# enijkamp/apex_example

Measured on AMD Instinct MI355X. Metric: images/sec (whole node) ResNet-50 amp O2, higher is better.
Workload: dtype bf16; 1 GPU; model=resnet50, global_batch=256, per_gpu_batch=256, image_size=224, parallelism=dp1, impl=amd, opt_level=O2, optimizer=FusedSGD(momentum=0.9, wd=5e-5), channels_last=True, fused_bn=True, syncbn=False, force_collectives=False, gemm_1x1=True, hip_graph=False, main_stream_priority=default, deterministic=False

## Files before the change

apex_example_amd/models/resnet.py:

```python
from __future__ import annotations

import weakref

import torch
import torch.nn as nn

from ..ops.batch_norm import BatchNorm2dReLU
from ..ops.batch_norm import bn_add_bn_relu
from ..ops.conv import Conv2d1x1, Conv2d3x3, StemConv2d, conv1x1_pair_s2
from ..ops.pool import (GlobalAvgPool2dNHWC, MaxPool2dNHWC, bn_relu_maxpool,
                        bn_relu_maxpool_fusable)


def conv3x3(in_planes, out_planes, stride=1, groups=1, dilation=1, mfma=False):
    if mfma and stride in (1, 2) and groups == 1 and dilation == 1:
        return Conv2d3x3(in_planes, out_planes, stride)
    return nn.Conv2d(in_planes, out_planes, kernel_size=3, stride=stride, padding=dilation,
                     groups=groups, bias=False, dilation=dilation)


def conv1x1(in_planes, out_planes, stride=1, gemm=False):
    if gemm:
        return Conv2d1x1(in_planes, out_planes, stride=stride)
    return nn.Conv2d(in_planes, out_planes, kernel_size=1, stride=stride, bias=False)
# ... 8 lines not shown
        if fused:
            self.bn = BatchNorm2dReLU(planes, fuse_relu=relu)
        else:
            self.bn = nn.BatchNorm2d(planes)
        if zero_init:
            nn.init.zeros_(self.bn.weight)

    def forward(self, x, z=None):
        if self.fused:
            return self.bn(x, z)
        y = self.bn(x)
        if z is not None:
            y = y + z
        return torch.relu(y) if self.relu_after else y


def _link_stats(conv, bnact):
    if bnact.fused:
        conv._amd_stats_bn = weakref.ref(bnact)


class BasicBlock(nn.Module):
    expansion = 1

    def __init__(self, inplanes, planes, stride=1, downsample=None, fused_bn=False,
                 zero_init_residual=False, gemm_1x1=False):
        super().__init__()
        self.conv1 = conv3x3(inplanes, planes, stride, mfma=gemm_1x1)
        self.bn1 = _BNAct(planes, True, fused_bn)
        self.conv2 = conv3x3(planes, planes, mfma=gemm_1x1)
        self.bn2 = _BNAct(planes, True, fused_bn, zero_init_residual)
        self.downsample = downsample
        _link_stats(self.conv1, self.bn1)
        _link_stats(self.conv2, self.bn2)

    def forward(self, x):
        identity = x if self.downsample is None else self.downsample(x)
        out = self.bn1(self.conv1(x))
        return self.bn2(self.conv2(out), identity)


class Bottleneck(nn.Module):
    expansion = 4

    def __init__(self, inplanes, planes, stride=1, downsample=None, fused_bn=False,
                 zero_init_residual=False, gemm_1x1=False):
        super().__init__()
        width = planes
        self.conv1 = conv1x1(inplanes, width, gemm=gemm_1x1)
        self.bn1 = _BNAct(width, True, fused_bn)
        self.conv2 = conv3x3(width, width, stride, mfma=gemm_1x1)
        self.bn2 = _BNAct(width, True, fused_bn)
        self.conv3 = conv1x1(width, planes * self.expansion, gemm=gemm_1x1)
        self.bn3 = _BNAct(planes * self.expansion, True, fused_bn, zero_init_residual)
        self.downsample = downsample
        _link_stats(self.conv1, self.bn1)
        _link_stats(self.conv2, self.bn2)
        _link_stats(self.conv3, self.bn3)

    def forward(self, x):
        fuse_ds = self.downsample is not None and self.bn3.fused and self.downsample.bn.fused
        proj = identity = None
        if (isinstance(self.conv1, Conv2d1x1) and self.downsample is not None
                and self.downsample.conv.stride == (2, 2)):
            out, proj = conv1x1_pair_s2(self.conv1, self.downsample.conv, x)
        elif isinstance(self.conv1, Conv2d1x1):
            out, skip = self.conv1.forward_with_skip(x)
            if self.downsample is None:
                identity = skip
            else:
                proj = self.downsample.conv(skip)
        else:
            if self.downsample is None:
                identity = x
            else:
                proj = self.downsample.conv(x)
            out = self.conv1(x)
        if proj is not None and not fuse_ds:
            identity = self.downsample.bn(proj)
        out = self.bn1(out)
        out = self.bn2(self.conv2(out))
        if proj is not None and fuse_ds:
            return bn_add_bn_relu(self.bn3.bn, self.conv3(out), self.downsample.bn.bn, proj)
        return self.bn3(self.conv3(out), identity)


class _Downsample(nn.Module):
    def __init__(self, inplanes, outplanes, stride, fused_bn, gemm_1x1=False):
        super().__init__()
        self.conv = conv1x1(inplanes, outplanes, stride, gemm=gemm_1x1)
        self.bn = _BNAct(outplanes, False, fused_bn)
        _link_stats(self.conv, self.bn)

    def forward(self, x):
        return self.bn(self.conv(x))


class ResNet(nn.Module):
    def __init__(self, block, layers, num_classes=1000, fused_bn=False, zero_init_residual=False,
                 gemm_1x1=False):
        super().__init__()
        self.fused_bn = fused_bn
        self.gemm_1x1 = gemm_1x1
        self.inplanes = 64
        if gemm_1x1 and self.inplanes == 64:
            self.conv1 = StemConv2d(3, self.inplanes)
        else:
            self.conv1 = nn.Conv2d(3, self.inplanes, kernel_size=7, stride=2, padding=3,
                                   bias=False)
        self.bn1 = _BNAct(self.inplanes, True, fused_bn)
        if isinstance(self.conv1, StemConv2d):
            _link_stats(self.conv1, self.bn1)
        pool = MaxPool2dNHWC if fused_bn else nn.MaxPool2d
        self.maxpool = pool(kernel_size=3, stride=2, padding=1)
        self.layer1 = self._make_layer(block, 64, layers[0], 1, zero_init_residual)
        self.layer2 = self._make_layer(block, 128, layers[1], 2, zero_init_residual)
        self.layer3 = self._make_layer(block, 256, layers[2], 2, zero_init_residual)
        self.layer4 = self._make_layer(block, 512, layers[3], 2, zero_init_residual)
        self.avgpool = GlobalAvgPool2dNHWC() if fused_bn else nn.AdaptiveAvgPool2d((1, 1))
        self.fc = nn.Linear(512 * block.expansion, num_classes)
        for m in self.modules():
            if isinstance(m, nn.Conv2d):
                nn.init.kaiming_normal_(m.weight, mode="fan_out", nonlinearity="relu")

    def _make_layer(self, block, planes, blocks, stride, zero_init_residual):
        downsample = None
        if stride != 1 or self.inplanes != planes * block.expansion:
            downsample = _Downsample(self.inplanes, planes * block.expansion, stride,
                                     self.fused_bn, self.gemm_1x1)
        layers = [block(self.inplanes, planes, stride, downsample, self.fused_bn,
                        zero_init_residual, self.gemm_1x1)]
        self.inplanes = planes * block.expansion
        for _ in range(1, blocks):
            layers.append(block(self.inplanes, planes, fused_bn=self.fused_bn,
                                zero_init_residual=zero_init_residual, gemm_1x1=self.gemm_1x1))
        return nn.Sequential(*layers)

    def forward(self, x):
        x = self.conv1(x)
        if (self.fused_bn and isinstance(self.maxpool, MaxPool2dNHWC)
                and bn_relu_maxpool_fusable(x, self.bn1.bn, self.maxpool)):
            x = bn_relu_maxpool(x, self.bn1.bn, self.maxpool)
        else:
            x = self.maxpool(self.bn1(x))
        x = self.layer1(x)
        x = self.layer2(x)
        x = self.layer3(x)
        x = self.layer4(x)
        x = self.avgpool(x)
        x = torch.flatten(x, 1)
        return self.fc(x)


def resnet18(**kw):
    return ResNet(BasicBlock, [2, 2, 2, 2], **kw)


def resnet34(**kw):
    return ResNet(BasicBlock, [3, 4, 6, 3], **kw)


def resnet50(**kw):
    return ResNet(Bottleneck, [3, 4, 6, 3], **kw)


def resnet101(**kw):
# ... 6 lines not shown
```

apex_example_amd/ops/batch_norm.py:

```python
from __future__ import annotations

import os
import threading

import torch
import torch.distributed as dist

from .. import _native
from . import _ddp_direct

_BWD_EPI = os.environ.get("APEX_AMD_CONV_BN_BWD", "1") == "1"
_TLS = threading.local()
FUSED_BWD_CALLS = [0]

_X2_BWD = os.environ.get("APEX_AMD_BN_X2", "1") == "1"
X2_BWD_CALLS = [0]


def _x2_target_ok(zc, ctx, weight):
    return (getattr(zc, "world", 0) == 1 and not getattr(zc, "fuse_relu", True)
            and not getattr(zc, "has_z", True) and getattr(zc, "count", -1) == ctx.count
            and not getattr(zc, "shape_channel_last", True) and not ctx.shape_channel_last
            and (zc.saved_tensors[2] is None) == (weight is None)
            and (weight is None or zc.saved_tensors[2].dtype == weight.dtype)
            and zc.saved_tensors[6] is None)


class BnBwdSrc:
    __slots__ = ("x", "mean", "invstd", "weight", "bias", "mask", "relu_mode", "result")

    def __init__(self, x, mean, invstd, weight, bias, mask, relu_mode):
        self.x, self.mean, self.invstd = x, mean, invstd
        self.weight, self.bias, self.mask, self.relu_mode = weight, bias, mask, relu_mode
        self.result = None


def _bwd_src(x, xl, mean, invstd, weight, bias, mask, fuse_relu, has_z):
    if not (_BWD_EPI and x.is_cuda and x.dtype == torch.bfloat16 and x.dim() == 4
            and x is xl and x.size(1) % 64 == 0
            and x.is_contiguous(memory_format=torch.channels_last)):
        return None
    if fuse_relu and has_z:
        if mask is None:
            return None
        mode = 1
    elif fuse_relu:
        if any(t is not None and t.dtype != torch.float32 for t in (weight, bias)):
            return None
        mode = 2
    else:
        mode = 0
    return BnBwdSrc(x, mean, invstd, weight, bias, mask, mode)


_RAW_RCCL = os.environ.get("APEX_AMD_SYNCBN_RAW_RCCL", "1") == "1"
_COMMS = {}


def _raw_comm(pg):
    return _raw_comm_rank(pg)[0]


def _raw_comm_rank(pg):
    if not _RAW_RCCL:
        return 0, -1
    c = _COMMS.get(id(pg))
    if c is not None and c[0] is pg:
        return c[1], c[2]
    from ..parallel.sync_batchnorm import is_syncbn_comm_group

    ptr = 0
    if is_syncbn_comm_group(pg) and _native.require().reducer.syncbn_raw_available():
        try:
            ptr = int(pg._get_backend(torch.device("cuda"))._comm_ptr())
        except Exception:
            ptr = 0
    rank = dist.get_rank(pg)
    if ptr:
        _COMMS[id(pg)] = (pg, ptr, rank)
    return ptr, rank


_SBN_EVENTS = None


def syncbn_timing(on=True):
    global _SBN_EVENTS
    _SBN_EVENTS = [] if on else None


def syncbn_timing_result():
    ev = _SBN_EVENTS
    if not ev:
        return None
    ev[-1][2].synchronize()
    out = {"calls": len(ev), "ms": 0.0, "allgather_ms": 0.0, "allreduce_ms": 0.0}
    for kind, a, b in ev:
        ms = a.elapsed_time(b)
        out["ms"] += ms
        out[kind + "_ms"] += ms
    return out


class _SbnTimer:
    def __init__(self, kind):
        self.kind = kind

    def __enter__(self):
        if _SBN_EVENTS is not None:
            self.a = torch.cuda.Event(enable_timing=True)
            self.a.record()
        return self

    def __exit__(self, *exc):
        if _SBN_EVENTS is not None and hasattr(self, "a"):
            b = torch.cuda.Event(enable_timing=True)
            b.record()
            _SBN_EVENTS.append((self.kind, self.a, b))
        return False


def _allreduce(t, pg):
    if t.is_cuda and _SBN_EVENTS is not None:
        with _SbnTimer("allreduce"):
            return _allreduce_body(t, pg)
    return _allreduce_body(t, pg)


def _allreduce_body(t, pg):
    if dist.get_backend(pg) == "nccl":
        comm = _raw_comm(pg)
        if comm:
            _native.require().reducer.syncbn_allreduce_raw(t, comm)
        else:
            _native.require().reducer.syncbn_allreduce(t, pg)
    else:
        dist.all_reduce(t, group=pg)


SLOT_GATHER_CALLS = [0]


def _gather_slot(C, world, rank, device):
    n = 2 * C + 1
    assert 0 <= rank < world, (rank, world)
    gathered = torch.empty(world * n, dtype=torch.float32, device=device)
    SLOT_GATHER_CALLS[0] += 1
    return gathered, gathered[rank * n:(rank + 1) * n]


def _direct_targets(params, need_w):
    direct = _ddp_direct.slots(*params) if need_w else None
    if direct is None:
        return None, None, None, True
    tw, aw = _ddp_direct.grad_target(params[0])
    tb, ab = _ddp_direct.grad_target(params[1])
    if aw != ab:
        return None, None, None, True
    return direct, tw, tb, aw


def bn_src_of(x):
    return getattr(x, "_amd_bn_src", None)


def _C():
    return _native.require().bn


def _to_logical(x, shape_channel_last):
    if shape_channel_last:
        C = x.size(-1)
        return x.reshape(-1, C)
    return x


class BatchNormFunction(torch.autograd.Function):
    @staticmethod
    def forward(ctx, x, z, weight, bias, running_mean, running_var, eps, momentum, process_group,
                fuse_relu, shape_channel_last, num_batches_tracked=None, force_collectives=False,
                slab=None, slab_shift=None):
        C = _C()
        ctx.params = (weight, bias)
        if ctx.needs_input_grad[2] or ctx.needs_input_grad[3]:
            _ddp_direct.note_use(weight, bias)
        orig_shape = x.shape
        xl = _to_logical(x, shape_channel_last)
        zl = _to_logical(z, shape_channel_last) if z is not None else None
        count = xl.numel() // xl.size(1)
        if process_group is False or not (dist.is_available() and dist.is_initialized()):
            world = 1
            force_collectives = False
        else:
            world = dist.get_world_size(process_group)
        collective = world > 1 or bool(force_collectives)
        want_mask = bool(fuse_relu) and zl is not None and xl.is_cuda
        if not collective and xl.is_cuda:
            if slab is not None:
                mean_g, invstd = C.slab_train_stats(slab, count, slab_shift, running_mean,
                                                    running_var, num_batches_tracked,
                                                    float(eps), float(momentum))
                if want_mask:
                    y, mask = C.apply_mask(xl, mean_g, invstd, weight, bias, zl, bool(fuse_relu))
                else:
                    y, mask = C.apply(xl, mean_g, invstd, weight, bias, zl, bool(fuse_relu)), None
            else:
                y, mean_g, invstd, mask = C.forward_local(xl, weight, bias, running_mean,
                                                          running_var, num_batches_tracked,
                                                          float(eps), float(momentum), zl,
                                                          bool(fuse_relu), want_mask)
            ctx.save_for_backward(xl, zl if mask is None else None, weight, bias, mean_g, invstd,
                                  mask)
            ctx.src = _TLS.src = _bwd_src(x, xl, mean_g, invstd, weight, bias, mask,
                                          bool(fuse_relu), zl is not None)
            ctx.pg, ctx.world, ctx.fuse_relu, ctx.total, ctx.count = None, 1, bool(fuse_relu), \
                None, count
            zg = getattr(z, "grad_fn", None) if z is not None else None
            ctx.zctx = zg if isinstance(zg, BatchNormFunction._backward_cls) else None
            ctx.pre = None
            ctx.orig_shape, ctx.has_z, ctx.shape_channel_last = orig_shape, z is not None, \
                shape_channel_last
            return y.view(orig_shape) if shape_channel_last else y
        if collective and xl.is_cuda:
            pg = process_group if process_group is not None else dist.group.WORLD
            nccl = dist.get_backend(pg) == "nccl"
            comm, rank = _raw_comm_rank(pg) if nccl else (0, dist.get_rank(pg))
            gathered = slot = None
            if comm or not nccl:
                gathered, slot = _gather_slot(xl.size(1), world, rank, x.device)
            packed = (C.slab_packed_stats(slab, count, slab_shift, out=slot) if slab is not None
                      else C.local_stats_packed(xl, out=slot))
            if nccl:
                R = _native.require().reducer
                with _SbnTimer("allgather"):
                    if comm:
                        mean_g, invstd, inv_total = R.syncbn_allgather_combine_raw(
                            packed, comm, world, float(eps), float(momentum), running_mean,
                            running_var, num_batches_tracked, gathered=gathered, rank=rank)
                    else:
                        mean_g, invstd, inv_total = R.syncbn_allgather_combine(
                            packed, pg, float(eps), float(momentum), running_mean,
                            running_var, num_batches_tracked)
            else:
                with _SbnTimer("allgather"):
                    dist.all_gather(list(gathered.chunk(world)), packed.clone(), group=pg)
                mean_g, invstd, inv_total = C.combine_stats_sync(
                    gathered.view(world, -1), float(eps), float(momentum), running_mean,
                    running_var, num_batches_tracked)
            if want_mask:
                y, mask = C.apply_mask(xl, mean_g, invstd, weight, bias, zl, bool(fuse_relu))
            else:
                y, mask = C.apply(xl, mean_g, invstd, weight, bias, zl, bool(fuse_relu)), None
            ctx.save_for_backward(xl, zl if mask is None else None, weight, bias, mean_g, invstd,
                                  mask)
            ctx.src = _TLS.src = _bwd_src(x, xl, mean_g, invstd, weight, bias, mask,
                                          bool(fuse_relu), zl is not None)
            ctx.pg, ctx.world, ctx.fuse_relu, ctx.total, ctx.count = pg, max(world, 2), \
                bool(fuse_relu), inv_total, count
            ctx.orig_shape, ctx.has_z, ctx.shape_channel_last = orig_shape, z is not None, \
                shape_channel_last
            return y.view(orig_shape) if shape_channel_last else y
        if num_batches_tracked is not None:
            num_batches_tracked.add_(1)
        mean, var = C.local_stats(xl)
        if collective:
            pg = process_group if process_group is not None else dist.group.WORLD
            cnt = torch.full((1,), float(count), dtype=torch.float32, device=x.device)
            packed = torch.cat([mean, var, cnt])
            gathered = torch.empty(world * packed.numel(), dtype=packed.dtype, device=x.device)
            dist.all_gather_into_tensor(gathered, packed, group=pg)
            g = gathered.view(world, -1)
            Cn = mean.numel()
            means, vars_, counts = g[:, :Cn], g[:, Cn:2 * Cn], g[:, 2 * Cn]
            total = counts.sum()
        else:
            pg = None
            means, vars_ = mean.view(1, -1), var.view(1, -1)
            counts = torch.full((1,), float(count), dtype=torch.float32, device=x.device)
            total = None
        mean_g, invstd, _ = C.combine_stats(means, vars_, counts, float(eps), float(momentum),
                                            running_mean, running_var)
        if want_mask:
            y, mask = C.apply_mask(xl, mean_g, invstd, weight, bias, zl, bool(fuse_relu))
        else:
            y, mask = C.apply(xl, mean_g, invstd, weight, bias, zl, bool(fuse_relu)), None
        ctx.save_for_backward(xl, zl if mask is None else None, weight, bias, mean_g, invstd, mask)
        ctx.src = None
        ctx.pg = pg
        ctx.world = max(world, 2) if collective else world
        ctx.fuse_relu = bool(fuse_relu)
        ctx.total = total
        ctx.count = count
        ctx.orig_shape = orig_shape
        ctx.has_z = z is not None
        ctx.shape_channel_last = shape_channel_last
        return y.view(orig_shape) if shape_channel_last else y

    @staticmethod
    def backward(ctx, dy):
        C = _C()
        xl, zl, weight, bias, mean, invstd, mask = ctx.saved_tensors
        dyl = _to_logical(dy, ctx.shape_channel_last)
        need_w = weight is not None and (ctx.needs_input_grad[2] or ctx.needs_input_grad[3])
        src = ctx.src
        res = src.result if src is not None else None
        if res is not None:
            src.result = None
        if res is not None and res[0] == dyl.data_ptr() and res[2] == dyl._version and (
                dyl.is_contiguous(memory_format=torch.channels_last)):
            FUSED_BWD_CALLS[0] += 1
            if ctx.world > 1:
                direct, tw, tb, acc = _direct_targets(ctx.params, need_w)
                sum_dy, sum_dy_xmu, gw, gb = C.slab_reduce_grad(res[1], invstd, weight, need_w,
                                                               sum_scale=ctx.total,
                                                               grad_weight=tw, grad_bias=tb,
                                                               accumulate=acc)
                if direct:
                    _ddp_direct.mark_ready(direct)
                    need_w = False
                n = sum_dy.numel()
                _allreduce(sum_dy.as_strided((2 * n,), (1,)), ctx.pg)
                total = 1.0
            else:
                sum_dy, sum_dy_xmu, gw, gb = C.slab_reduce_grad(res[1], invstd, weight, need_w)
                total = float(ctx.count)
            zc = getattr(ctx, "zctx", None) if ctx.has_z else None
            if _X2_BWD and zc is not None and ctx.world == 1 and _x2_target_ok(zc, ctx, weight):
                xd, _, wd, _, md, isd, _ = zc.saved_tensors
                if C.backward_x2_ok(dyl, xl, xd):
                    need_wd = wd is not None and (zc.needs_input_grad[2] or zc.needs_input_grad[3])
                    dx, s1, s2, gw2, gb2 = C.backward_elemt_x2(
                        dyl, xl, mean, invstd, weight, bias, sum_dy, sum_dy_xmu, total, xd, md,
                        isd, wd, need_wd)
                    zc.pre = (dyl.data_ptr(), dyl._version, s1, s2, gw2, gb2)
                    return (dx, dyl, gw if need_w else None, gb if need_w else None, None, None,
                            None, None, None, None, None, None, None, None, None)
            dx, _ = C.backward_elemt(dyl, xl, mean, invstd, weight, bias, sum_dy, sum_dy_xmu,
                                     total, None, False, False)
            return (dx, dyl if ctx.has_z else None, gw if need_w else None,
                    gb if need_w else None, None, None, None, None, None, None, None, None, None,
                    None, None)
        pre = getattr(ctx, "pre", None)
        if pre is not None:
            ctx.pre = None
            if pre[0] == dyl.data_ptr() and pre[1] == dyl._version:
                _, _, sum_dy, sum_dy_xmu, gw, gb = pre
                X2_BWD_CALLS[0] += 1
                dx, _ = C.backward_elemt(dyl, xl, mean, invstd, weight, bias, sum_dy, sum_dy_xmu,
                                         float(ctx.count), None, False, False)
                if ctx.shape_channel_last:
                    dx = dx.view(ctx.orig_shape)
                return (dx, None, gw if need_w else None, gb if need_w else None, None, None,
                        None, None, None, None, None, None, None, None, None)
        if ctx.world > 1 and xl.is_cuda:
            direct, tw, tb, acc = _direct_targets(ctx.params, need_w)
            sum_dy, sum_dy_xmu, gw, gb = C.reduce_grad(dyl, xl, mean, invstd, weight, bias, zl,
                                                       ctx.fuse_relu, need_w, mask=mask,
                                                       sum_scale=ctx.total, grad_weight=tw,
                                                       grad_bias=tb, accumulate=acc)
            if direct:
                _ddp_direct.mark_ready(direct)
                need_w = False
            n = sum_dy.numel()
            packed = sum_dy.as_strided((2 * n,), (1,))
            _allreduce(packed, ctx.pg)
            dx, dz = C.backward_elemt(dyl, xl, mean, invstd, weight, bias, sum_dy, sum_dy_xmu,
                                      1.0, zl, ctx.fuse_relu, ctx.has_z, mask=mask)
            if ctx.shape_channel_last:
                dx = dx.view(ctx.orig_shape)
                if dz is not None:
                    dz = dz.view(ctx.orig_shape)
            return (dx, dz if ctx.has_z else None, gw if need_w else None,
                    gb if need_w else None, None, None, None, None, None, None, None, None, None, None, None)
        if ctx.world == 1 and xl.is_cuda:
            dx, dz, gw, gb = C.backward_local(dyl, xl, mean, invstd, weight, bias, zl,
                                              ctx.fuse_relu, need_w, ctx.has_z, mask=mask)
            if ctx.shape_channel_last:
                dx = dx.view(ctx.orig_shape)
                if dz is not None:
                    dz = dz.view(ctx.orig_shape)
            return (dx, dz if ctx.has_z else None, gw if need_w else None,
                    gb if need_w else None, None, None, None, None, None, None, None, None, None, None, None)
        sum_dy, sum_dy_xmu, gw, gb = C.reduce_grad(dyl, xl, mean, invstd, weight, bias, zl,
                                                   ctx.fuse_relu, need_w, mask=mask)
        if ctx.world > 1:
            packed = torch.cat([sum_dy, sum_dy_xmu])
            dist.all_reduce(packed, group=ctx.pg)
            n = sum_dy.numel()
            packed = packed / ctx.total
            sum_dy, sum_dy_xmu = packed[:n], packed[n:]
            total = 1.0
        else:
            total = float(ctx.count)
        dx, dz = C.backward_elemt(dyl, xl, mean, invstd, weight, bias, sum_dy, sum_dy_xmu, total,
                                  zl, ctx.fuse_relu, ctx.has_z, mask=mask)
        if ctx.shape_channel_last:
            dx = dx.view(ctx.orig_shape)
            if dz is not None:
                dz = dz.view(ctx.orig_shape)
        return (dx, dz if ctx.has_z else None, gw if need_w else None, gb if need_w else None,
                None, None, None, None, None, None, None, None, None, None, None)


def take_slab(x, bn):
    ent = getattr(x, "_amd_bn_stats", None)
    if ent is None:
        return None, None
    del x._amd_bn_stats
    slab, shift, owner = ent
    if owner is not bn or slab.size(1) != x.size(1):
        return None, None
    return slab, shift


def batch_norm_act(x, weight, bias, running_mean, running_var, training, momentum, eps,
                   z=None, fuse_relu=False, process_group=False, shape_channel_last=False,
                   num_batches_tracked=None, force_collectives=False, slab=None, slab_shift=None):
    if training:
        _TLS.src = None
        y = BatchNormFunction.apply(x, z, weight, bias, running_mean, running_var, eps, momentum,
                                    process_group, fuse_relu, shape_channel_last,
                                    num_batches_tracked, force_collectives, slab, slab_shift)
        src = _TLS.src
        if src is not None:
            _TLS.src = None
            y._amd_bn_src = src
        return y
    if shape_channel_last:
        xs = x.movedim(-1, 1)
        zs = z.movedim(-1, 1) if z is not None else None
    else:
        xs, zs = x, z
    y = torch.nn.functional.batch_norm(xs, running_mean, running_var, weight, bias, False, 0.0, eps)
    if zs is not None:
        y = y + zs
    if fuse_relu:
        y = torch.relu(y)
    return y.movedim(1, -1) if shape_channel_last else y


class BatchNorm2dReLU(torch.nn.BatchNorm2d):

    def __init__(self, num_features, eps=1e-5, momentum=0.1, affine=True,
                 track_running_stats=True, fuse_relu=True, **kw):
        super().__init__(num_features, eps, momentum, affine, track_running_stats, **kw)
        self.fuse_relu = fuse_relu

    def _amd_accepts_slab(self):
        return self.training and (self.momentum is not None or not self.track_running_stats)

    def forward(self, x, z=None):
        slab, shift = take_slab(x, self)
        if not x.is_cuda and not _native.available():
            y = super().forward(x)
            if z is not None:
                y = y + z
            return torch.relu(y) if self.fuse_relu else y
        momentum = 0.0 if self.momentum is None else self.momentum
        nbt = None
        if self.training and self.track_running_stats:
            if self.momentum is None:
                self.num_batches_tracked.add_(1)
                momentum = 1.0 / float(self.num_batches_tracked)
            else:
                nbt = self.num_batches_tracked
        use_batch = self.training or not self.track_running_stats
        return batch_norm_act(x, self.weight, self.bias,
                              self.running_mean if self.track_running_stats else None,
                              self.running_var if self.track_running_stats else None,
                              use_batch, momentum, self.eps, z=z, fuse_relu=self.fuse_relu,
                              process_group=False, num_batches_tracked=nbt,
                              slab=slab if use_batch else None, slab_shift=shift)


_FUSE_DS = os.environ.get("APEX_AMD_BN_DS_FUSE", "1") == "1"
FUSED_DS_CALLS = [0]


class BatchNormAddBNReLUFunction(torch.autograd.Function):
    @staticmethod
    def forward(ctx, x, xd, w, b, wd, bd, rm, rv, nbt, rmd, rvd, nbtd, eps, mom, epsd, momd,
                slab, shift, slabd, shiftd):
        C = _C()
        ctx.params = (w, b, wd, bd)
        if ctx.needs_input_grad[2] or ctx.needs_input_grad[3]:
            _ddp_direct.note_use(w, b)
        if ctx.needs_input_grad[4] or ctx.needs_input_grad[5]:
            _ddp_direct.note_use(wd, bd)
        count = x.numel() // x.size(1)

        def stats(t, sl, sh, rm_, rv_, nbt_, eps_, mom_):
            if sl is not None:
                return C.slab_train_stats(sl, count, sh, rm_, rv_, nbt_, float(eps_), float(mom_))
            return C.train_stats(t, rm_, rv_, nbt_, float(eps_), float(mom_))

        mean, invstd = stats(x, slab, shift, rm, rv, nbt, eps, mom)
        meand, invstdd = stats(xd, slabd, shiftd, rmd, rvd, nbtd, epsd, momd)
        y, mask = C.apply2_mask(x, mean, invstd, w, b, xd, meand, invstdd, wd, bd)
        ctx.save_for_backward(x, xd, w, b, wd, bd, mean, invstd, meand, invstdd, mask)
        ctx.src = _TLS.src = _bwd_src(x, x, mean, invstd, w, b, mask, True, True)
        ctx.count = count
        FUSED_DS_CALLS[0] += 1
        return y

    @staticmethod
    def backward(ctx, dy):
        C = _C()
        x, xd, w, b, wd, bd, mean, invstd, meand, invstdd, mask = ctx.saved_tensors
        need = w is not None and (ctx.needs_input_grad[2] or ctx.needs_input_grad[3])
        needd = wd is not None and (ctx.needs_input_grad[4] or ctx.needs_input_grad[5])
        cnt = float(ctx.count)
        src = ctx.src
        res = src.result if src is not None else None
        if res is not None:
            src.result = None
        if (res is not None and res[0] == dy.data_ptr() and res[2] == dy._version
                and dy.is_contiguous(memory_format=torch.channels_last)):
            FUSED_BWD_CALLS[0] += 1
            s1, s2, gw, gb = C.slab_reduce_grad(res[1], invstd, w, need)
            dx, t1, t2, gwd, gbd = C.backward_elemt_x2(dy, x, mean, invstd, w, b, s1, s2, cnt,
                                                       xd, meand, invstdd, wd, needd)
            dxd, _ = C.backward_elemt(dy, xd, meand, invstdd, wd, bd, t1, t2, cnt, None, False,
                                      False)
        else:
            dyc = dy.contiguous(memory_format=torch.channels_last)
            s1, s2, gw, gb = C.reduce_grad(dyc, x, mean, invstd, w, b, None, True, need,
                                           mask=mask)
            dx, d = C.backward_elemt(dyc, x, mean, invstd, w, b, s1, s2, cnt, None, True, True,
                                     mask=mask)
            dxd, _, gwd, gbd = C.backward_local(d, xd, meand, invstdd, wd, bd, None, False,
                                                needd, False)
        return (dx, dxd, gw if need else None, gb if need else None, gwd if needd else None,
                gbd if needd else None) + (None,) * 14


def _ds_fusable(bn, x, bnd, xd):
    return (_FUSE_DS and type(bn) is BatchNorm2dReLU and type(bnd) is BatchNorm2dReLU
            and bn.training and bnd.training and bn.fuse_relu and not bnd.fuse_relu
            and bn.track_running_stats and bnd.track_running_stats
            and bn.momentum is not None and bnd.momentum is not None
            and bn.affine == bnd.affine and x.is_cuda and xd.is_cuda and x.dim() == 4
            and x.shape == xd.shape and x.dtype == xd.dtype
            and x.dtype in (torch.bfloat16, torch.float16)
            and (not bn.affine or bn.weight.dtype == bnd.weight.dtype)
            and _native.available() and _C().backward_x2_ok(x, x, xd))


def bn_add_bn_relu(bn, x, bnd, xd):
    if not _ds_fusable(bn, x, bnd, xd):
        return bn(x, bnd(xd))
    slab, shift = take_slab(x, bn)
    slabd, shiftd = take_slab(xd, bnd)
    _TLS.src = None
    y = BatchNormAddBNReLUFunction.apply(
        x, xd, bn.weight, bn.bias, bnd.weight, bnd.bias, bn.running_mean, bn.running_var,
# ... 8 lines not shown
```

apex_example_amd/ops/conv.py:

```python
from __future__ import annotations

import collections
import os
import threading

import torch
import torch.nn as nn
import torch.nn.functional as F

from .. import _native
from . import _ddp_direct
from .batch_norm import bn_src_of

_USE_WSTREAM = os.environ.get("APEX_AMD_WGRAD_STREAM", "1") == "1"
_SIDE = {}
_JOIN = {}
_LOCK = threading.Lock()


def _ddp_slot(p):
    return _ddp_direct.slot(p)


def _side_mode(params):
    ps = [p for p in params if p is not None]
    if not _USE_WSTREAM or not ps or not ps[0].is_cuda:
        return None
    if torch.cuda.is_current_stream_capturing():
        return None
    if all(p.grad is None for p in ps) and not any(
            getattr(p, "_amd_grad_is_bucket_view", False) for p in ps):
        import torch.distributed as dist
        if dist.is_available() and dist.is_initialized() and dist.get_world_size() > 1:
            return None
        return "free"
    if _DDP_SIDE and all(_ddp_slot(p) is not None for p in ps):
        return "ddp"
    return None


_DDP_SIDE = os.environ.get("APEX_AMD_WGRAD_STREAM_DDP", "1") == "1"
_SIDE_EVENTS = {}


_TEST_SIDE_SLEEP = 0


def _join_side():
    with _LOCK:
        pending = list(_JOIN.items())
        _JOIN.clear()
        for idx, _ in pending:
            _SIDE_EVENTS.pop(idx, None)
    for idx, (main, _task) in pending:
        for key, side in list(_SIDE.items()):
            if key[0] == idx:
                main.wait_stream(side)


def _lag_for(mode):
    return 4 if mode == "ddp" else 0


def join_side_streams():
    _join_side()


class _SideWgrad:

    def __init__(self, weight, *more, enable=True):
        self.params = (weight,) + more
        self.mode = _side_mode(self.params) if enable else None
        self.on = self.mode is not None
        if self.on:
            dev = weight.device
            self.main = torch.cuda.current_stream(dev)
            high = self.mode == "ddp"
            key = (dev.index, high)
            self.side = _SIDE.get(key)
            if self.side is None:
                prio = torch.cuda.Stream.priority_range()[1] if high else 0
                self.side = torch.cuda.Stream(dev, priority=prio)
                _SIDE[key] = self.side
            self.ev = self.main.record_event()

    def run(self, fn, *used):
        if not self.on:
            return fn()
        self.side.wait_event(self.ev)
        with torch.cuda.stream(self.side):
            if _TEST_SIDE_SLEEP:
                torch.cuda._sleep(_TEST_SIDE_SLEEP)
            dw = fn()
            outs = dw if isinstance(dw, tuple) else (dw,)
            if self.mode == "ddp":
# ... 142 lines not shown
            return got
        return _native.require().conv.transpose_weight(weight)
    return weight.reshape(co, ci).t().contiguous().view(ci, co, 1, 1)


def _conv1x1_dgrad(dy, weight, xshape):
    n, ci, h, w = xshape
    co = weight.shape[0]
    if _own_1x1(dy.dtype, co, ci, n * h * w) and weight.dtype == torch.bfloat16:
        return _native.require().conv.conv_fwd(dy, _transpose_1x1(weight), 1)
    dx2 = torch.mm(_as_rows(dy), weight.reshape(co, ci))
    return dx2.view(n, h, w, ci).permute(0, 3, 1, 2)


def _as_rows(t):
    n, c, h, w = t.shape
    return t.permute(0, 2, 3, 1).reshape(n * h * w, c)


_CONV_BN_STATS = os.environ.get("APEX_AMD_CONV_BN_STATS", "1") == "1"
_TLS = threading.local()


def _stats_bn(conv, x):
    if not (_CONV_BN_STATS and x.is_cuda and x.dtype == torch.bfloat16):
        return None
    link = getattr(conv, "_amd_stats_bn", None)
    owner = link() if link is not None else None
    bn = getattr(owner, "bn", None) if owner is not None else None
    if bn is None or not bn.training or not hasattr(bn, "_amd_accepts_slab"):
        return None
    if not bn._amd_accepts_slab():
        return None
    return bn


def _shift_of(bn):
    rm = bn.running_mean if bn.track_running_stats else None
    if rm is not None and rm.dtype == torch.float32 and rm.is_contiguous():
        return rm
    return None


def _conv_fwd(x, weight, stride, bn):
    cv = _native.require().conv
    if bn is None:
        return cv.conv_fwd(x, weight, stride)
    shift = _shift_of(bn)
    y, slab = cv.conv_fwd_stats(x, weight, stride, shift)
    _TLS.slab = (slab, shift, bn)
    return y


def _tag_stats(y):
    ent = getattr(_TLS, "slab", None)
    if ent is not None:
        _TLS.slab = None
        y._amd_bn_stats = ent
    return y




_BNBWD_MAX_M = int(os.environ.get("APEX_AMD_BNBWD_MAX_M", str((1 << 31) - 1)))
_BNBWD_S2 = os.environ.get("APEX_AMD_BNBWD_S2", "0") == "1"


def _bnbwd_ok(dy, weight, src, xshape, has_add=False):
    m = xshape[0] * xshape[2] * xshape[3]
    return (src is not None and dy.is_cuda and dy.dtype == torch.bfloat16
            and weight.dtype == torch.bfloat16 and tuple(src.x.shape) == tuple(xshape)
            and dy.size(1) % 64 == 0 and xshape[1] % 64 == 0 and m < (1 << 31)
            and (has_add or m <= _BNBWD_MAX_M) and _native.available())


def _dgrad_bn(dy, wprep, add, src, add_stride2=False):
    g, slab = _native.require().conv.conv_fwd_bnbwd(
        dy, wprep, add, src.x, src.mask, src.mean, src.invstd, src.weight, src.bias,
        src.relu_mode, add_stride2)
    src.result = (g.data_ptr(), slab, g._version)
    return g


class Conv1x1GemmFunction(torch.autograd.Function):
    @staticmethod
    def forward(ctx, x, weight, bn=None, src=None):
        ctx.save_for_backward(x, weight)
        ctx.src = src
        if ctx.needs_input_grad[1]:
            _ddp_direct.note_use(weight)
        n, ci, h, w = x.shape
        if ctx.needs_input_grad[0] and weight.dtype == torch.bfloat16 and (
                src is not None or _own_1x1(x.dtype, weight.shape[0], ci, n * h * w)):
            _register_prep(weight)
        return _conv1x1_fwd(x, weight, bn)

    @staticmethod
    def backward(ctx, dy):
        x, weight = ctx.saved_tensors
        dy = dy.contiguous(memory_format=torch.channels_last)
        dx = dw = None
        side = _SideWgrad(weight) if ctx.needs_input_grad[1] else None
        if ctx.needs_input_grad[0]:
            if _bnbwd_ok(dy, weight, ctx.src, x.shape):
                dx = _dgrad_bn(dy, _transpose_1x1(weight), None, ctx.src)
            else:
                dx = _conv1x1_dgrad(dy, weight, x.shape)
        ctx.src = None
        if ctx.needs_input_grad[1]:
            direct = None if side.on else _ddp_direct.slots(weight)
            tgt, acc = _ddp_direct.grad_target(weight) if direct is not None else (None, True)
            if direct is not None and tgt.is_contiguous():
                wgrad_1x1(_as_rows(dy), _as_rows(x), weight.dtype, out=tgt, accumulate=acc)
                _ddp_direct.mark_ready(direct)
            else:
                so, sa = _side_out(side, weight)
                dw = side.run(lambda: _wgrad_1x1_w(dy, x, weight, so, sa), dy, x)
        return dx, dw, None, None


class Conv1x1SkipFunction(torch.autograd.Function):

    @staticmethod
    def forward(ctx, x, weight, bn=None, src=None):
        ctx.save_for_backward(x, weight)
        ctx.src = src
        if ctx.needs_input_grad[1]:
            _ddp_direct.note_use(weight)
        if src is not None and ctx.needs_input_grad[0] and weight.dtype == torch.bfloat16:
            _register_prep(weight)
        return _conv1x1_fwd(x, weight, bn), x.view_as(x)

    @staticmethod
    def backward(ctx, dy, dskip):
        x, weight = ctx.saved_tensors
        n, ci, h, w = x.shape
        co = weight.shape[0]
        dx = dw = None
        if dy is not None:
            dy = dy.contiguous(memory_format=torch.channels_last)
        side = _SideWgrad(weight) if (ctx.needs_input_grad[1] and dy is not None) else None
        src, ctx.src = ctx.src, None
        if ctx.needs_input_grad[0]:
            if dy is None:
                dx = dskip
            elif _bnbwd_ok(dy, weight, src, x.shape, has_add=dskip is not None) and (
                    dskip is None or (dskip.dtype == torch.bfloat16 and dskip.shape == x.shape)):
                add = (dskip.contiguous(memory_format=torch.channels_last)
                       if dskip is not None else None)
                dx = _dgrad_bn(dy, _transpose_1x1(weight), add, src)
            else:
                w2 = weight.reshape(co, ci)
                if dskip is not None:
                    dskip = dskip.contiguous(memory_format=torch.channels_last)
                    dx2 = _as_rows(dskip).addmm_(_as_rows(dy), w2)
                else:
                    dx2 = torch.mm(_as_rows(dy), w2)
                dx = dx2.view(n, h, w, ci).permute(0, 3, 1, 2)
        if ctx.needs_input_grad[1] and dy is not None:
            direct = None if side.on else _ddp_direct.slots(weight)
            tgt, acc = _ddp_direct.grad_target(weight) if direct is not None else (None, True)
            if direct is not None and tgt.is_contiguous():
                wgrad_1x1(_as_rows(dy), _as_rows(x), weight.dtype, out=tgt, accumulate=acc)
                _ddp_direct.mark_ready(direct)
            else:
                so, sa = _side_out(side, weight)
                dw = side.run(lambda: _wgrad_1x1_w(dy, x, weight, so, sa), dy, x)
        return dx, dw, None, None


class Conv1x1Stride2Function(torch.autograd.Function):

    @staticmethod
    def forward(ctx, x, weight, bn=None):
        ctx.save_for_backward(x, weight)
        if ctx.needs_input_grad[1]:
            _ddp_direct.note_use(weight)
        if ctx.needs_input_grad[0]:
            _register_prep(weight)
        return _conv_fwd(x, weight, 2, bn)

    @staticmethod
    def backward(ctx, dy):
        x, weight = ctx.saved_tensors
        cv = _native.require().conv
        dy = dy.contiguous(memory_format=torch.channels_last)
        co, ci = weight.shape[0], weight.shape[1]
        dx = dw = None
        side = _SideWgrad(weight) if ctx.needs_input_grad[1] else None
        if ctx.needs_input_grad[0]:
            dx = cv.conv_dgrad_s2(dy, _transpose_1x1(weight), x.size(2), x.size(3))
        if ctx.needs_input_grad[1]:
            direct = None if side.on else _ddp_direct.slots(weight)
            tgt, acc = _ddp_direct.grad_target(weight) if direct is not None else (None, True)
            if direct is not None and tgt.is_contiguous(memory_format=torch.channels_last):
                cv.conv_wgrad(dy, x, weight.dtype, 0, 2, 1, out=tgt, accumulate=acc)
                _ddp_direct.mark_ready(direct)
            else:
                so, sa = _side_out(side, weight, cl=True)
                dw = side.run(lambda: cv.conv_wgrad(dy, x, weight.dtype, 0, 2, 1, out=so,
                                                    accumulate=sa), dy, x)
# ... 26 lines not shown
        return y1, yd

    @staticmethod
    def backward(ctx, dy1, dyd):
        x, w1, wd = ctx.saved_tensors
        n, ci, h, w = x.shape
        cv = _native.require().conv
        src, ctx.src = ctx.src, None
        dx = dw1 = dwd = None
        if dy1 is not None:
            dy1 = dy1.contiguous(memory_format=torch.channels_last)
        if dyd is not None:
            dyd = dyd.contiguous(memory_format=torch.channels_last)
        side1 = _SideWgrad(w1) if (ctx.needs_input_grad[1] and dy1 is not None) else None
        sided = _SideWgrad(wd) if (ctx.needs_input_grad[2] and dyd is not None) else None
        if ctx.needs_input_grad[0]:
            cd = (_conv1x1_dgrad(dyd, wd, (n, ci, h // 2, w // 2)).contiguous(
                memory_format=torch.channels_last) if dyd is not None else None)
            if dy1 is None:
                dx = torch.zeros_like(x)
                if cd is not None:
                    dx[:, :, ::2, ::2] = cd
            elif cd is not None and _bnbwd_ok(dy1, w1, src, x.shape, has_add=True):
                PAIR_S2_CALLS[0] += 1
                dx = _dgrad_bn(dy1, _transpose_1x1(w1), cd, src, add_stride2=True)
            else:
                dx = _conv1x1_dgrad(dy1, w1, x.shape).contiguous(
                    memory_format=torch.channels_last)
                if cd is not None:
                    dx[:, :, ::2, ::2] += cd
        if side1 is not None:
            direct = None if side1.on else _ddp_direct.slots(w1)
            tgt, acc = _ddp_direct.grad_target(w1) if direct is not None else (None, True)
            if direct is not None and tgt.is_contiguous():
                wgrad_1x1(_as_rows(dy1), _as_rows(x), w1.dtype, out=tgt, accumulate=acc)
                _ddp_direct.mark_ready(direct)
            else:
                so, sa = _side_out(side1, w1)
                dw1 = side1.run(lambda: _wgrad_1x1_w(dy1, x, w1, so, sa), dy1, x)
        if sided is not None:
            direct = None if sided.on else _ddp_direct.slots(wd)
            tgt, acc = _ddp_direct.grad_target(wd) if direct is not None else (None, True)
            if direct is not None and tgt.is_contiguous(memory_format=torch.channels_last):
                cv.conv_wgrad(dyd, x, wd.dtype, 0, 2, 1, out=tgt, accumulate=acc)
                _ddp_direct.mark_ready(direct)
            else:
                so, sa = _side_out(sided, wd, cl=True)
                dwd = sided.run(lambda: cv.conv_wgrad(dyd, x, wd.dtype, 0, 2, 1, out=so,
                                                      accumulate=sa), dyd, x)
        return dx, dw1, dwd, None, None, None


def conv1x1_pair_s2(conv1, convd, x):
    if (_PAIR_S2 and isinstance(conv1, Conv2d1x1) and isinstance(convd, Conv2d1x1)
            and conv1._gemm_ok(x) and convd._strided_ok(x) and x.dtype == torch.bfloat16
            and conv1.weight.dtype == torch.bfloat16 and _native.available()):
        y1, yd = Conv1x1PairS2Function.apply(x, conv1.weight, convd.weight,
                                             _stats_bn(conv1, x), _stats_bn(convd, x),
                                             bn_src_of(x))
        ent1, ent2 = getattr(_TLS, "pair", (None, None))
        _TLS.pair = (None, None)
        if ent1 is not None:
            y1._amd_bn_stats = ent1
        if ent2 is not None:
            yd._amd_bn_stats = ent2
        return y1, yd
    return conv1(x), convd(x)


class Conv2d1x1(nn.Conv2d):

    def __init__(self, in_planes, out_planes, stride=1, bias=False):
        super().__init__(in_planes, out_planes, kernel_size=1, stride=stride, bias=bias)

    def forward(self, x):
        if self._gemm_ok(x):
            return _tag_stats(Conv1x1GemmFunction.apply(x, self.weight, _stats_bn(self, x),
                                                        bn_src_of(x)))
        if self._strided_ok(x):
            return _tag_stats(Conv1x1Stride2Function.apply(x, self.weight, _stats_bn(self, x)))
        return F.conv2d(x, self.weight, self.bias, self.stride, self.padding, self.dilation,
                        self.groups)

    def forward_with_skip(self, x):
        if self._gemm_ok(x):
            y, skip = Conv1x1SkipFunction.apply(x, self.weight, _stats_bn(self, x),
                                                bn_src_of(x))
            return _tag_stats(y), skip
        return self.forward(x), x

    def _strided_ok(self, x):
        return (self.stride == (2, 2) and self.bias is None and x.is_cuda and x.dim() == 4
                and x.dtype == torch.bfloat16 and self.weight.dtype == torch.bfloat16
                and x.is_contiguous(memory_format=torch.channels_last) and self.groups == 1
                and x.size(2) % 2 == 0 and x.size(3) % 2 == 0
                and x.size(0) * x.size(2) * x.size(3) < (1 << 22)
                and self.in_channels % 64 == 0 and self.out_channels % 64 == 0)

    def _gemm_ok(self, x):
        return (self.stride == (1, 1) and self.bias is None and x.is_cuda and x.dim() == 4
                and x.is_contiguous(memory_format=torch.channels_last)
                and x.dtype == self.weight.dtype and self.groups == 1)


_WGRAD3 = "tap"
_WGRAD64 = True
_WGRAD9_ALL = os.environ.get("APEX_AMD_WGRAD9", "0") == "1"


def _wgrad3_algo(x, weight, stride):
    cin, cout = x.size(1), weight.size(0)
    if not (_WGRAD64 and stride == 1 and x.size(3) <= 56 and cin % 64 == 0
            and cout % 64 == 0):
        return 0
    if cin == 64 and cout == 64:
        return 4
    return 4 if _WGRAD9_ALL and x.size(3) >= 14 else 0
_USE_SPLITK_REDUCE = True
_USE_ROT_KERNEL = True


def _rot_weight(weight):
    if _USE_ROT_KERNEL and weight.is_cuda and weight.element_size() == 2:
        got = _prepared(weight)
        if got is not None:
            return got
        return _native.require().conv.rot_weight(weight)
    return weight.flip(2, 3).transpose(0, 1).contiguous(memory_format=torch.channels_last)


_USE_PREP = True
_PREP_PENDING = {}
_PREP_READY = {}


def _register_prep(weight):
    if not (_USE_PREP and weight.is_cuda and weight.element_size() == 2):
        return
    k = id(weight)
    _PREP_READY.pop(k, None)
    _PREP_PENDING[k] = weight


def _prepared(weight):
    k = id(weight)
    ent = _PREP_READY.get(k)
    if ent is not None and ent[0] is weight:
        return ent[1]
    if k not in _PREP_PENDING:
        return None
    ws = list(_PREP_PENDING.values())
    _PREP_PENDING.clear()
    _PREP_READY.clear()
    outs = _native.require().conv.prep_weights(ws)
    for w, o in zip(ws, outs):
        _PREP_READY[id(w)] = (w, o)
    return _PREP_READY[k][1]


class Conv3x3Function(torch.autograd.Function):

    @staticmethod
    def forward(ctx, x, weight, stride, bn=None, src=None):
        ctx.save_for_backward(x, weight)
        ctx.stride = stride
        ctx.src = src if stride == 1 else None
# ... 127 lines not shown
```

csrc/hip/bn_nhwc.hip:

```cpp
#include <cstdio>
#include <cstdlib>

#include "bn_common.h"

namespace amd {

namespace {

struct NGeom {
  int ctile, rows_iter, cblocks;
};

NGeom ngeom(int64_t C, bool vec) {
  NGeom g;
  int64_t cv = vec ? C / 8 : C;
  g.ctile = (int)(cv < 64 ? cv : 64);
  if (g.ctile < 1) g.ctile = 1;
  g.rows_iter = kBNThreads / g.ctile;
  g.cblocks = (int)((cv + g.ctile - 1) / g.ctile);
  return g;
}

}

// ... 132 lines not shown
  float k[W], s1[W], s2[W];
#pragma unroll
  for (int i = 0; i < W; ++i) k[i] = s1[i] = s2[i] = 0.f;
  if (active) {
    ldw<T, W>(x + c0, k);
    for (int64_t r = r0 + ri; r < r1; r += (int64_t)rows_iter * U) {
      float v[U][W];
#pragma unroll
      for (int u = 0; u < U; ++u) {
        const int64_t rr = r + (int64_t)u * rows_iter;
#pragma unroll
        for (int i = 0; i < W; ++i) v[u][i] = k[i];
        if (rr < r1) ldw<T, W>(x + rr * C + c0, v[u]);
      }
#pragma unroll
      for (int u = 0; u < U; ++u)
#pragma unroll
        for (int i = 0; i < W; ++i) {
          const float d = v[u][i] - k[i];
          s1[i] += d;
          s2[i] = fmaf(d, d, s2[i]);
        }
    }
  }
  block_slab_write<W>(s1, s2, ci, ri, ctile, rows_iter, c0, C, slab);
}

constexpr int kBNBlockChans = 64 * 8;

template <typename F>
__device__ __forceinline__ void stage_params(int C, int cb, int n, F&& f) {
  const int lim = cb + n < C ? n : C - cb;
  for (int k = threadIdx.x; k < lim; k += blockDim.x) f(cb + k, k);
  __syncthreads();
}

template <typename T, typename TW, bool VEC, int U, bool ZZ, bool ZA = false>
__global__ void __launch_bounds__(kBNThreads)
    apply_k(const T* __restrict__ x, const float* __restrict__ mean,
            const float* __restrict__ invstd, const TW* __restrict__ w, const TW* __restrict__ b,
            const T* __restrict__ z, T* __restrict__ y, uint8_t* __restrict__ rmask, int64_t M,
            int C, int ctile, int rows_iter, int relu, const float* __restrict__ meanz = nullptr,
            const float* __restrict__ invstdz = nullptr, const TW* __restrict__ wz = nullptr,
            const TW* __restrict__ bz = nullptr) {
  constexpr int W = VEC ? 8 : 1;
  const int Cb = C >> 3;
  const int ci = threadIdx.x % ctile, ri = threadIdx.x / ctile;
  const int c0 = (blockIdx.y * ctile + ci) * W;
  __shared__ __attribute__((aligned(16))) float s_par[ZA ? 4 : 2][kBNBlockChans];
  const int cb = blockIdx.y * ctile * W;
  stage_params(C, cb, ctile * W, [&](int c, int k) {
    chan_affine(mean, invstd, wload(w, c, 1.f), wload(b, c, 0.f), c, s_par[0][k], s_par[1][k]);
    if constexpr (ZA)
      chan_affine(meanz, invstdz, wload(wz, c, 1.f), wload(bz, c, 0.f), c, s_par[ZA ? 2 : 0][k],
                  s_par[ZA ? 3 : 1][k]);
  });
  if (ri >= rows_iter || c0 >= C) return;
  float sc[W], sh[W], scz[W], shz[W];
#pragma unroll
  for (int i = 0; i < W; ++i) {
    sc[i] = s_par[0][c0 - cb + i];
    sh[i] = s_par[1][c0 - cb + i];
    scz[i] = ZA ? s_par[ZA ? 2 : 0][c0 - cb + i] : 0.f;
    shz[i] = ZA ? s_par[ZA ? 3 : 1][c0 - cb + i] : 0.f;
  }
  const int64_t stride = (int64_t)gridDim.x * rows_iter;
  for (int64_t r = (int64_t)blockIdx.x * rows_iter + ri; r < M; r += stride * U) {
    float v[U][W], zz[U][W];
#pragma unroll
    for (int u = 0; u < U; ++u) {
      const int64_t rr = r + (int64_t)u * stride;
      const int64_t rc = rr < M ? rr : M - 1;
      ldw<T, W>(x + rc * C + c0, v[u]);
      if constexpr (ZZ) ldw<T, W>(z + rc * C + c0, zz[u]);
    }
    asm volatile("" ::: "memory");
#pragma unroll
    for (int u = 0; u < U; ++u) {
      const int64_t rr = r + (int64_t)u * stride;
      if (rr >= M) continue;
      uint32_t mb = 0;
#pragma unroll
      for (int i = 0; i < W; ++i) {
        float o = fmaf(v[u][i], sc[i], sh[i]);
        if constexpr (ZA) {
          o += to_f32(from_f32<T>(fmaf(zz[u][i], scz[i], shz[i])));
        } else if constexpr (ZZ) {
          o += zz[u][i];
        }
        mb |= (o > 0.f ? 1u : 0u) << i;
        v[u][i] = relu ? fmaxf(o, 0.f) : o;
      }
      stw<T, W>(y + rr * C + c0, v[u]);
      if constexpr (W == 8) {
        if (rmask) rmask[rr * Cb + (c0 >> 3)] = (uint8_t)mb;
      }
    }
  }
}

template <typename T, typename TW, bool VEC, int U, int RM>
__global__ void __launch_bounds__(kBNThreads)
    reduce_k(const T* __restrict__ dy, const T* __restrict__ x, const float* __restrict__ mean,
             const float* __restrict__ invstd, const TW* __restrict__ w, const TW* __restrict__ b,
             const T* __restrict__ z, const uint8_t* __restrict__ rmask, int64_t M,
             int C, int ctile, int rows_iter, float* __restrict__ slab) {
  constexpr int W = VEC ? 8 : 1;
  const int Cb = C >> 3;
  const int ci = threadIdx.x % ctile, ri = threadIdx.x / ctile;
  const int c0 = (blockIdx.y * ctile + ci) * W;
  const bool active = ri < rows_iter && c0 < C;
  const int64_t per = (M + gridDim.x - 1) / gridDim.x;
  const int64_t r0 = (int64_t)blockIdx.x * per;
  const int64_t r1 = r0 + per < M ? r0 + per : M;
  float mu[W], sc[W], sh[W], s1[W], s2[W];
#pragma unroll
  for (int i = 0; i < W; ++i) mu[i] = sc[i] = sh[i] = s1[i] = s2[i] = 0.f;
  __shared__ __attribute__((aligned(16))) float s_par[3][kBNBlockChans];
  const int cb = blockIdx.y * ctile * W;
  stage_params(C, cb, ctile * W, [&](int c, int k) {
    s_par[0][k] = mean[c];
    chan_affine(mean, invstd, wload(w, c, 1.f), wload(b, c, 0.f), c, s_par[1][k], s_par[2][k]);
  });
  if (active) {
#pragma unroll
    for (int i = 0; i < W; ++i) {
      const int k = c0 - cb + i;
      mu[i] = s_par[0][k];
      sc[i] = s_par[1][k];
      sh[i] = s_par[2][k];
    }
    for (int64_t r = r0 + ri; r < r1; r += (int64_t)rows_iter * U) {
      float xv[U][W], dv[U][W], zv[U][W];
      uint32_t mk[U];
      bool ok[U];
#pragma unroll
      for (int u = 0; u < U; ++u) {
        const int64_t rr = r + (int64_t)u * rows_iter;
        ok[u] = rr < r1;
        const int64_t rc = ok[u] ? rr : r1 - 1;
        ldw<T, W>(x + rc * C + c0, xv[u]);
        ldw<T, W>(dy + rc * C + c0, dv[u]);
        mk[u] = 0;
        if constexpr (RM == 1) mk[u] = rmask[rc * Cb + (c0 >> 3)];
        if constexpr (RM == 2) ldw<T, W>(z + rc * C + c0, zv[u]);
      }
#pragma unroll
      for (int u = 0; u < U; ++u)
#pragma unroll
        for (int i = 0; i < W; ++i) {
          float d = dv[u][i];
          if constexpr (RM == 1) {
            d = ((mk[u] >> ((c0 + i) & 7)) & 1u) ? d : 0.f;
          } else if constexpr (RM >= 2) {
            float o = fmaf(xv[u][i], sc[i], sh[i]);
            if constexpr (RM == 2) o += zv[u][i];
            d = o > 0.f ? d : 0.f;
          }
          d = ok[u] ? d : 0.f;
          const float xe = ok[u] ? xv[u][i] : 0.f;
          s1[i] += d;
          s2[i] = fmaf(d, xe - mu[i], s2[i]);
        }
    }
  }
  block_slab_write<W>(s1, s2, ci, ri, ctile, rows_iter, c0, C, slab);
}

template <typename T, typename TW, bool VEC, int U, int RM, bool X2 = false>
__global__ void __launch_bounds__(kBNThreads)
    backward_k(const T* __restrict__ dy, const T* __restrict__ x, const float* __restrict__ mean,
               const float* __restrict__ invstd, const TW* __restrict__ w,
               const TW* __restrict__ b, const float* __restrict__ sum_dy,
               const float* __restrict__ sum_dy_xmu, float inv_n,
               const T* __restrict__ z, const uint8_t* __restrict__ rmask, T* __restrict__ dx,
               T* __restrict__ dz, int64_t M, int C, int ctile, int rows_iter,
               const T* __restrict__ x2 = nullptr, const float* __restrict__ mean2 = nullptr,
               float* __restrict__ slab2 = nullptr) {
  constexpr int W = VEC ? 8 : 1;
  const int Cb = C >> 3;
  const int ci = threadIdx.x % ctile, ri = threadIdx.x / ctile;
  const int c0 = (blockIdx.y * ctile + ci) * W;
  __shared__ __attribute__((aligned(16))) float s_par[X2 ? 6 : 5][kBNBlockChans];
  const int cb = blockIdx.y * ctile * W;
  stage_params(C, cb, ctile * W, [&](int c, int k) {
    const float wc = wload(w, c, 1.f);
    chan_affine(mean, invstd, wc, wload(b, c, 0.f), c, s_par[0][k], s_par[1][k]);
    const float is = invstd[c];
    const float mdy = sum_dy[c] * inv_n, mdyx = sum_dy_xmu[c] * inv_n;
    const float q1 = is * wc, q2 = -is * is * is * wc * mdyx;
    s_par[2][k] = q1;
    s_par[3][k] = q2;
    s_par[4][k] = -is * wc * mdy - q2 * mean[c];
    if constexpr (X2) s_par[X2 ? 5 : 0][k] = mean2[c];
  });
  float t1[W], t2[W], m2[W];
#pragma unroll
  for (int i = 0; i < W; ++i) t1[i] = t2[i] = m2[i] = 0.f;
  const bool active = ri < rows_iter && c0 < C;
  if (!X2 && !active) return;
  float sc[W], sh[W], k1[W], k2[W], k3[W];
#pragma unroll
  for (int i = 0; i < W; ++i) {
    const int k = active ? c0 - cb + i : 0;
    sc[i] = s_par[0][k];
    sh[i] = s_par[1][k];
    k1[i] = s_par[2][k];
    k2[i] = s_par[3][k];
    k3[i] = s_par[4][k];
    if constexpr (X2) m2[i] = s_par[X2 ? 5 : 0][k];
  }
  const int64_t stride = (int64_t)gridDim.x * rows_iter;
  for (int64_t r = (int64_t)blockIdx.x * rows_iter + ri; active && r < M; r += stride * U) {
    float xv[U][W], dv[U][W], zv[U][W], x2v[X2 ? U : 1][W];
    uint32_t mk[U];
#pragma unroll
    for (int u = 0; u < U; ++u) {
      const int64_t rr = r + (int64_t)u * stride;
      const int64_t rc = rr < M ? rr : M - 1;
      mk[u] = 0;
      ldw<T, W>(x + rc * C + c0, xv[u]);
      ldw<T, W>(dy + rc * C + c0, dv[u]);
      if constexpr (RM == 1) mk[u] = rmask[rc * Cb + (c0 >> 3)];
      if constexpr (RM == 2) ldw<T, W>(z + rc * C + c0, zv[u]);
      if constexpr (X2) ldw<T, W>(x2 + rc * C + c0, x2v[u]);
    }
    asm volatile("" ::: "memory");
#pragma unroll
    for (int u = 0; u < U; ++u) {
      const int64_t rr = r + (int64_t)u * stride;
      if (rr >= M) continue;
#pragma unroll
      for (int i = 0; i < W; ++i) {
        float d = dv[u][i];
        if constexpr (RM == 1) {
          d = ((mk[u] >> ((c0 + i) & 7)) & 1u) ? d : 0.f;
        } else if constexpr (RM >= 2) {
          float o = fmaf(xv[u][i], sc[i], sh[i]);
          if constexpr (RM == 2) o += zv[u][i];
          d = o > 0.f ? d : 0.f;
        }
        dv[u][i] = d;
        xv[u][i] = fmaf(d, k1[i], fmaf(xv[u][i], k2[i], k3[i]));
        if constexpr (X2) {
          t1[i] += d;
          t2[i] = fmaf(d, x2v[u][i] - m2[i], t2[i]);
        }
      }
      stw<T, W>(dx + rr * C + c0, xv[u]);
      if (dz) stw<T, W>(dz + rr * C + c0, dv[u]);
    }
  }
  if constexpr (X2) block_slab_write_cm<W>(t1, t2, ci, ri, ctile, rows_iter, c0, C, slab2);
}


constexpr int kSlabPerThread = 16;

static int slab_ch(int S) {
  int ch = 1;
  while (ch < 32 && (int64_t)S * ch * 2 <= (int64_t)kBNThreads * kSlabPerThread) ch *= 2;
  return ch;
}

template <int CH>
__device__ __forceinline__ void slab_t_sum(const float* __restrict__ slab, int S, int C, int c0,
                                           float* out) {
  constexpr int TPC = kBNThreads / CH;
  __shared__ float red[2][kBNThreads];
  const int k = threadIdx.x / TPC, t = threadIdx.x - k * TPC;
  const int c = c0 + k;
  float a[8], b[8];
#pragma unroll
  for (int u = 0; u < 8; ++u) a[u] = b[u] = 0.f;
  if (c < C) {
    const float* r0 = slab + (int64_t)c * S;
    const float* r1 = slab + (int64_t)(C + c) * S;
    int s = t;
    for (; s + 7 * TPC < S; s += 8 * TPC) {
      float va[8], vb[8];
#pragma unroll
      for (int u = 0; u < 8; ++u) {
        va[u] = r0[s + u * TPC];
        vb[u] = r1[s + u * TPC];
      }
#pragma unroll
      for (int u = 0; u < 8; ++u) {
        a[u] += va[u];
        b[u] += vb[u];
      }
    }
    for (; s < S; s += TPC) {
      a[0] += r0[s];
      b[0] += r1[s];
    }
  }
  red[0][threadIdx.x] = ((a[0] + a[1]) + (a[2] + a[3])) + ((a[4] + a[5]) + (a[6] + a[7]));
  red[1][threadIdx.x] = ((b[0] + b[1]) + (b[2] + b[3])) + ((b[4] + b[5]) + (b[6] + b[7]));
  __syncthreads();
#pragma unroll
  for (int w = TPC / 2; w > 0; w >>= 1) {
    if (t < w) {
      red[0][threadIdx.x] += red[0][threadIdx.x + w];
      red[1][threadIdx.x] += red[1][threadIdx.x + w];
    }
    __syncthreads();
  }
  if (t == 0) {
    out[k] = red[0][threadIdx.x];
    out[CH + k] = red[1][threadIdx.x];
  }
  __syncthreads();
}

template <int CH>
__global__ void __launch_bounds__(kBNThreads)
    slab_stats_k(const float* __restrict__ slab, int S, int C, int64_t count,
                 const float* __restrict__ shift, BNStatsOut out) {
  __shared__ float sums[2 * CH];
  const int c0 = blockIdx.x * CH;
  slab_t_sum<CH>(slab, S, C, c0, sums);
  const int k = threadIdx.x;
  if (k < CH && c0 + k < C) {
    const int c = c0 + k;
    const float sh = shift ? shift[c] : 0.f;
    const double m = (double)sums[k] / (double)count;
// ... 298 lines not shown
```

csrc/hip/conv_igemm.hip:

```cpp
#include <algorithm>
#include <cstdlib>
#include <cstring>
#include <type_traits>

#include "amd_dev.h"
#include "amd_kernels.h"

namespace amd {

namespace {

typedef float f32x4_t __attribute__((ext_vector_type(4)));

constexpr int kCT = 256;
constexpr int kBM = 128;
constexpr int kBK = 64;
constexpr int kRowBytes = kBK * 2;

__device__ uint4 g_zero16[4];

__device__ __forceinline__ int swz(int row, int chunk) {
  return row * kRowBytes + ((chunk ^ ((row >> 1) & 7)) << 4);
}

template <int RB>
__device__ __forceinline__ int swz_key(int row) {
  if constexpr (RB == 128) return (row >> 1) & 7;
  else return ((row >> 2) & 1) << 1;
}
template <int RB>
__device__ __forceinline__ int swzr(int row, int chunk) {
  return row * RB + ((chunk ^ swz_key<RB>(row)) << 4);
}

__device__ __forceinline__ void glds16(const void* g, unsigned char* l) {
  __builtin_amdgcn_global_load_lds((const __attribute__((address_space(1))) void*)g,
                                   (__attribute__((address_space(3))) void*)l, 16, 0, 0);
}

__device__ __forceinline__ void glds16a(const void* g, unsigned char* l) {
#if defined(__HIP_DEVICE_COMPILE__)
  const uint32_t la = (uint32_t)(uintptr_t)(__attribute__((address_space(3))) unsigned char*)l;
  asm volatile("global_load_lds_dwordx4 %0, off" : : "v"(g), "{m0}"(la) : "memory");
#endif
}

__device__ __forceinline__ void lds_barrier() {
  asm volatile("s_waitcnt lgkmcnt(0)" ::: "memory");
  __builtin_amdgcn_s_barrier();
  asm volatile("" ::: "memory");
}

__device__ __forceinline__ int xcd_remap(int bid, int nwg) {
  const int xcd = bid % 8, q = nwg / 8, r = nwg % 8;
  const int base = xcd < r ? xcd * (q + 1) : r * (q + 1) + (xcd - r) * q;
  return base + bid / 8;
}

enum ConvMode { kFwd3 = 0, kFwd1 = 1, kDgrad3 = 2, kDgrad1 = 3 };

template <int MODE>
__device__ __forceinline__ int conv_ntaps(int z) {
  if constexpr (MODE == kFwd3) return 9;
  else if constexpr (MODE == kFwd1) return 1;
  else if constexpr (MODE == kDgrad3) return ((z >> 1) ? 2 : 1) * ((z & 1) ? 2 : 1);
  else return z == 0 ? 1 : 0;
}

template <int MODE>
__device__ __forceinline__ void conv_tap(int z, int t, int& dh, int& dw, int& wt) {
  if constexpr (MODE == kFwd3) {
    const int r = t / 3, s = t - r * 3;
    dh = r - 1; dw = s - 1; wt = t;
  } else if constexpr (MODE == kDgrad3) {
    const int ph = z >> 1, pw = z & 1, ns = pw ? 2 : 1;
    const int ri = t / ns, si = t - ri * ns;
    const int r = ph ? 2 * ri : 1, s = pw ? 2 * si : 1;
    dh = (ph + 1 - r) >> 1; dw = (pw + 1 - s) >> 1;
    wt = 8 - (3 * r + s);
  } else {
    dh = 0; dw = 0; wt = 0;
  }
}

struct ConvGeom {
  int GH, GW, AH, AW, as, YH, YW, ys, KC, NC, M, kb_stride;
};

template <int BM, int BN, int CT = kCT>
// ... 64 lines not shown
      const int h = rem / g.GW, w = rem - h * g.GW;
      aoff = ((int64_t)(n * (g.GH >> 1) + (h >> 1)) * (g.GW >> 1) + (w >> 1)) * NC + c0;
      a_on = ((h | w) & 1) == 0;
    }
    P.av[q] = *reinterpret_cast<const uint4*>(a_on ? addp + aoff : zb);
    P.xv[q] = *reinterpret_cast<const uint4*>(x_on ? xp + off : zb);
    P.mk[q] = *(rm1 ? ep.rmask + opix * (NC >> 3) + (c0 >> 3) : g_ff16);
  }
}

template <int MODE, int BM, int BN, int CT, int RM, bool ADD, int TS>
__device__ __forceinline__ void bnbwd_store_t(const bf16_t* T, bf16_t* __restrict__ y,
                                              const ConvGeom& g, int m0, int n0, int z,
                                              const BnPre<BM, BN, CT>& P, float (&s1)[8],
                                              float (&s2)[8]) {
  using PT = BnPre<BM, BN, CT>;
  const int tid = threadIdx.x;
  const int cc = tid % PT::CPR, rg = tid / PT::CPR;
  const int c0 = n0 + cc * 8;
  __builtin_amdgcn_s_waitcnt(0x0F70);
  float sc[8], sh[8];
#pragma unroll
  for (int i = 0; i < 8; ++i) {
    sc[i] = P.iv[i] * P.wv[i];
    sh[i] = P.bv[i] - P.mu[i] * sc[i];
  }
#pragma unroll
  for (int q = 0; q < PT::ROWS; ++q) {
    const int row = q * PT::RGS + rg;
    const int m = m0 + row;
    if (m >= g.M) continue;
    const uint4 tv = *reinterpret_cast<const uint4*>(T + row * TS + cc * 8);
    const unsigned tw[4] = {tv.x, tv.y, tv.z, tv.w};
    const unsigned aw[4] = {P.av[q].x, P.av[q].y, P.av[q].z, P.av[q].w};
    const unsigned xw[4] = {P.xv[q].x, P.xv[q].y, P.xv[q].z, P.xv[q].w};
    unsigned ow[4];
#pragma unroll
    for (int k = 0; k < 4; ++k) {
      float o[2], xx[2];
      o[0] = __uint_as_float(tw[k] << 16);
      o[1] = __uint_as_float(tw[k] & 0xffff0000u);
      if constexpr (ADD) {
        o[0] += __uint_as_float(aw[k] << 16);
        o[1] += __uint_as_float(aw[k] & 0xffff0000u);
      }
      xx[0] = __uint_as_float(xw[k] << 16);
      xx[1] = __uint_as_float(xw[k] & 0xffff0000u);
      unsigned short hb[2];
#pragma unroll
      for (int h = 0; h < 2; ++h) {
        const int i = 2 * k + h;
        bool keep = true;
        if constexpr (RM == 1) keep = (P.mk[q] >> i) & 1u;
        else if constexpr (RM == 2) keep = fmaf(xx[h], sc[i], sh[i]) > 0.f;
        const bf16_t gb = (bf16_t)(keep ? o[h] : 0.f);
        const float gv = (float)gb;
        s1[i] += gv;
        s2[i] = fmaf(gv, xx[h] - P.mu[i], s2[i]);
        hb[h] = __builtin_bit_cast(unsigned short, gb);
      }
      ow[k] = (unsigned)hb[0] | ((unsigned)hb[1] << 16);
    }
    *reinterpret_cast<uint4*>(y + out_pix<MODE>(g, m, z) * g.NC + c0) =
        make_uint4(ow[0], ow[1], ow[2], ow[3]);
  }
}

template <int MODE, int BM, int BN, int CT, int TS>
__device__ __forceinline__ void bnbwd_store(const bf16_t* T, bf16_t* __restrict__ y,
                                            const ConvGeom& g, const ConvBnEpi& ep, int m0,
                                            int n0, int z, const BnPre<BM, BN, CT>& P,
                                            float (&s1)[8], float (&s2)[8]) {
  const bool add = ep.add != nullptr;
  switch (ep.relu_mode * 2 + (add ? 1 : 0)) {
    case 0: bnbwd_store_t<MODE, BM, BN, CT, 0, false, TS>(T, y, g, m0, n0, z, P, s1, s2); break;
    case 1: bnbwd_store_t<MODE, BM, BN, CT, 0, true, TS>(T, y, g, m0, n0, z, P, s1, s2); break;
    case 2: bnbwd_store_t<MODE, BM, BN, CT, 1, false, TS>(T, y, g, m0, n0, z, P, s1, s2); break;
    case 3: bnbwd_store_t<MODE, BM, BN, CT, 1, true, TS>(T, y, g, m0, n0, z, P, s1, s2); break;
    case 4: bnbwd_store_t<MODE, BM, BN, CT, 2, false, TS>(T, y, g, m0, n0, z, P, s1, s2); break;
    default: bnbwd_store_t<MODE, BM, BN, CT, 2, true, TS>(T, y, g, m0, n0, z, P, s1, s2); break;
  }
}

template <int MODE, int BM, int BN, int WM, int WN, int NB, int EPI = 0, int CT = kCT,
          int BK = kBK, bool EARLY = false>
__global__ void __launch_bounds__(CT, (NB * (BM + BN) * BK * 2 > 80 * 1024)
                                          ? 1 : (NB == 1 && EPI == 0 ? 3 : 2))
    conv_tap_k(const bf16_t* __restrict__ x, const bf16_t* __restrict__ wt,
               bf16_t* __restrict__ y, ConvGeom g, float* __restrict__ slab,
               const float* __restrict__ shift, ConvBnEpi ep) {
  constexpr int NW = CT / 64;
  static_assert(WM * WN == NW, "one wave per output sub-tile");
  constexpr int TM = BM / WM, TN = BN / WN;
  constexpr int FM = TM / 16, FN = TN / 16;
  constexpr int RB = BK * 2;
  constexpr int LPR = RB / 16;
  constexpr int RPI = 64 / LPR;
  constexpr int KS = BK / 32;
  constexpr int A_BYTES = BM * RB, B_BYTES = BN * RB;
  constexpr int BUF = A_BYTES + B_BYTES;
  constexpr int AI = BM / (RPI * NW);
  constexpr int BI = BN / (RPI * NW);
  static_assert(AI >= 1 && BI >= 1, "tile rows per wave");
  constexpr int G = AI + BI;
  constexpr int TS = BN + 8;
  constexpr int EPI_BYTES = BM * TS * 2 > 2 * CT * 8 * 4 ? BM * TS * 2 : 2 * CT * 8 * 4;
  constexpr int LDS_BYTES = NB * BUF > EPI_BYTES ? NB * BUF : EPI_BYTES;
  __shared__ __attribute__((aligned(1024))) unsigned char lds[LDS_BYTES];

  const int tid = threadIdx.x, lane = tid & 63, wid = tid >> 6;
  const int wm = wid / WN, wn = wid % WN;
  const int NTf = gridDim.y == 1 ? g.NC / BN : 1;
  const int lt = xcd_remap(blockIdx.x, gridDim.x);
  const int mt = lt / NTf, MTn = (int)gridDim.x / NTf;
  const int m0 = mt * BM, n0 = (gridDim.y == 1 ? lt - mt * NTf : (int)blockIdx.y) * BN;
  const int z = MODE == kDgrad3 ? (int)gridDim.z - 1 - (int)blockIdx.z : (int)blockIdx.z;
  const int ntaps = conv_ntaps<MODE>(z);
  const int KC = g.KC, M = g.M, GHW = g.GH * g.GW;

  const int lrow = lane / LPR, pchunk = lane % LPR;
  const bf16_t* abase[AI];
  unsigned amask[AI];
#pragma unroll
  for (int q = 0; q < AI; ++q) {
    const int row = wid * (BM / NW) + q * RPI + lrow;
    const int ch = pchunk ^ swz_key<RB>(row);
    const int m = m0 + row;
    const int mm = m < M ? m : 0;
    const int n = mm / GHW;
    const int rem = mm - n * GHW;
    const int gh = rem / g.GW, gw = rem - gh * g.GW;
    const int h = gh * g.as, w = gw * g.as;
    abase[q] = x + ((int64_t)(n * g.AH + h) * g.AW + w) * KC + ch * 8;
    unsigned mk = 0;
    constexpr int TMAX = MODE == kFwd3 ? 9 : (MODE == kDgrad3 ? 4 : 1);
#pragma unroll
    for (int t = 0; t < TMAX; ++t) {
      int dh, dw, wti;
      conv_tap<MODE>(z, t, dh, dw, wti);
      const int hh = h + dh, ww = w + dw;
      if (t < ntaps && m < M && hh >= 0 && hh < g.AH && ww >= 0 && ww < g.AW) mk |= 1u << t;
    }
    amask[q] = mk;
  }
  const bf16_t* bbase[BI];
#pragma unroll
  for (int q = 0; q < BI; ++q) {
    const int row = wid * (BN / NW) + q * RPI + lrow;
    bbase[q] = wt + (int64_t)(n0 + row) * g.kb_stride + (pchunk ^ swz_key<RB>(row)) * 8;
  }
  const int kc_per_tap = KC / BK;
  const int KT = ntaps * kc_per_tap;

#define CONV_ISSUE(kt_)                                                                     \
  {                                                                                         \
                                 \
    const int tap_ = (MODE == kFwd1 || MODE == kDgrad1) ? 0 : (kt_) / kc_per_tap;           \
    const int c0_ = ((kt_) - tap_ * kc_per_tap) * BK;                                       \
    int dh_, dw_, wt_;                                                                      \
    conv_tap<MODE>(z, tap_, dh_, dw_, wt_);                                                 \
    const int64_t aoff_ = (int64_t)(dh_ * g.AW + dw_) * KC + c0_;                           \
    const int boff_ = wt_ * KC + c0_;                                                       \
    unsigned char* A_ = lds + ((kt_) % NB) * BUF;                                           \
    unsigned char* B_ = A_ + A_BYTES;                                                       \
    _Pragma("unroll") for (int q = 0; q < AI; ++q) {                                        \
      const bool ok = (amask[q] >> tap_) & 1u;                                              \
      glds16(ok ? (const void*)(abase[q] + aoff_) : (const void*)g_zero16,                  \
             A_ + (wid * (BM / NW) + q * RPI) * RB);                                       \
    }                                                                                       \
    _Pragma("unroll") for (int q = 0; q < BI; ++q)                                          \
      glds16(bbase[q] + boff_, B_ + (wid * (BN / NW) + q * RPI) * RB);                      \
  }

  f32x4_t acc[FM][FN];
#pragma unroll
  for (int i = 0; i < FM; ++i)
#pragma unroll
    for (int j = 0; j < FN; ++j) acc[i][j] = f32x4_t{0.f, 0.f, 0.f, 0.f};

  const int fr = lane & 15, fg = lane >> 4;
  constexpr int CPR = BN / 8;
  const bool want_stats = EPI == 1 ? slab != nullptr
                                   : (MODE == kFwd3 || MODE == kFwd1) && slab != nullptr;
  const int scc = tid % CPR;
  float shv[8];
#pragma unroll
  for (int i = 0; i < 8; ++i)
    shv[i] = (EPI == 0 && want_stats && shift) ? shift[n0 + scc * 8 + i] : 0.f;

  BnPre<BM, BN, CT> pre;
  if constexpr (EPI == 1 && EARLY) bnbwd_prefetch<MODE, BM, BN, CT>(g, ep, m0, n0, z, pre);

  {
  #pragma unroll
    for (int p = 0; p < NB - 1; ++p)
      if (p < KT) CONV_ISSUE(p);

    for (int kt = 0; kt < KT; ++kt) {
      if constexpr (NB == 1) {
        if (kt > 0) __syncthreads();
        CONV_ISSUE(kt);
        asm volatile("s_waitcnt vmcnt(0)" ::: "memory");
        __builtin_amdgcn_s_barrier();
      } else {
        if (kt + NB - 2 < KT) {
          asm volatile("s_waitcnt vmcnt(%0)" ::"n"(G * (NB > 2 ? NB - 2 : 0)) : "memory");
        } else {
          asm volatile("s_waitcnt vmcnt(0)" ::: "memory");
        }
        __builtin_amdgcn_s_barrier();
        asm volatile("" ::: "memory");
        if (kt + NB - 1 < KT) CONV_ISSUE(kt + NB - 1);
      }
      const unsigned char* A = lds + (kt % NB) * BUF;
      const unsigned char* B = A + A_BYTES;
  #pragma unroll
      for (int ks = 0; ks < KS; ++ks) {
        const int ch = ks * 4 + fg;
        bf16x8 af[FM], bfr[FN];
  #pragma unroll
        for (int i = 0; i < FM; ++i)
          af[i] = *reinterpret_cast<const bf16x8*>(A + swzr<RB>(wm * TM + i * 16 + fr, ch));
  #pragma unroll
        for (int j = 0; j < FN; ++j)
          bfr[j] = *reinterpret_cast<const bf16x8*>(B + swzr<RB>(wn * TN + j * 16 + fr, ch));
  #pragma unroll
        for (int i = 0; i < FM; ++i)
  #pragma unroll
          for (int j = 0; j < FN; ++j)
            acc[i][j] = __builtin_amdgcn_mfma_f32_16x16x32_bf16(bfr[j], af[i], acc[i][j], 0, 0, 0);
      }
    }
  }
#undef CONV_ISSUE
  if constexpr (EPI == 1) {
    if constexpr (!EARLY) bnbwd_prefetch<MODE, BM, BN, CT>(g, ep, m0, n0, z, pre);
    lds_barrier();
  } else {
    __syncthreads();
  }

  bf16_t* T = reinterpret_cast<bf16_t*>(lds);
#pragma unroll
  for (int i = 0; i < FM; ++i)
#pragma unroll
    for (int j = 0; j < FN; ++j) {
      const int row = wm * TM + i * 16 + fr;
      const int col = wn * TN + j * 16 + fg * 4;
      const unsigned lo = (unsigned)__builtin_bit_cast(unsigned short, (bf16_t)acc[i][j][0]) |
                          ((unsigned)__builtin_bit_cast(unsigned short, (bf16_t)acc[i][j][1]) << 16);
      const unsigned hi = (unsigned)__builtin_bit_cast(unsigned short, (bf16_t)acc[i][j][2]) |
                          ((unsigned)__builtin_bit_cast(unsigned short, (bf16_t)acc[i][j][3]) << 16);
      *reinterpret_cast<uint2*>(T + row * TS + col) = make_uint2(lo, hi);
    }
  if constexpr (EPI == 1) {
    lds_barrier();
  } else {
    __syncthreads();
  }
  constexpr bool dense = MODE == kFwd3 || MODE == kFwd1;
  float s1[8], s2[8];
#pragma unroll
  for (int i = 0; i < 8; ++i) s1[i] = s2[i] = 0.f;
  if constexpr (EPI == 1) {
    bnbwd_store<MODE, BM, BN, CT, TS>(T, y, g, ep, m0, n0, z, pre, s1, s2);
  } else
  for (int c = tid; c < BM * CPR; c += CT) {
    const int row = c / CPR, cc = c - row * CPR;
    const int m = m0 + row;
    if (m >= M) continue;
    int64_t opix = m;
    if (!dense) {
      const int n = m / GHW;
      const int rem = m - n * GHW;
      const int gh = rem / g.GW, gw = rem - gh * g.GW;
      opix = (int64_t)(n * g.YH + gh * g.ys + (z >> 1)) * g.YW + gw * g.ys + (z & 1);
    }
    const uint4 v = *reinterpret_cast<const uint4*>(T + row * TS + cc * 8);
    *reinterpret_cast<uint4*>(y + opix * g.NC + n0 + cc * 8) = v;
    if (want_stats) {
      const unsigned wv[4] = {v.x, v.y, v.z, v.w};
#pragma unroll
      for (int q = 0; q < 4; ++q) {
        const float lo = __uint_as_float(wv[q] << 16) - shv[2 * q];
        const float hi = __uint_as_float(wv[q] & 0xffff0000u) - shv[2 * q + 1];
        s1[2 * q] += lo;
        s2[2 * q] = fmaf(lo, lo, s2[2 * q]);
        s1[2 * q + 1] += hi;
        s2[2 * q + 1] = fmaf(hi, hi, s2[2 * q + 1]);
      }
    }
  }
  if (want_stats) {
    constexpr int RGS = CT / CPR;
    lds_barrier();
    float* red = reinterpret_cast<float*>(lds);
    const int rg = tid / CPR;
#pragma unroll
    for (int i = 0; i < 8; ++i) {
      red[rg * BN + scc * 8 + i] = s1[i];
      red[RGS * BN + rg * BN + scc * 8 + i] = s2[i];
    }
    lds_barrier();
    if (tid < BN) {
      float a = 0.f, b = 0.f;
#pragma unroll 4
      for (int q = 0; q < RGS; ++q) {
        a += red[q * BN + tid];
        b += red[RGS * BN + q * BN + tid];
      }
      const int64_t S = (int64_t)MTn * gridDim.z, s = (int64_t)z * MTn + mt;
      slab[(int64_t)(n0 + tid) * S + s] = a;
      slab[(int64_t)(g.NC + n0 + tid) * S + s] = b;
    }
  }
}

int g_bnbwd_early = 1;

int g_conv_nfast = 1;

inline dim3 conv_grid(int mtiles, int ntiles, int nclasses, bool one_by_one) {
  (void)one_by_one;
  const bool fold = ntiles > 1 && (g_conv_nfast == 2 ||
                                   (g_conv_nfast == 1 && !(ntiles == 4 && mtiles >= 1024)));
  return fold ? dim3((unsigned)(mtiles * ntiles), 1, nclasses)
              : dim3((unsigned)mtiles, (unsigned)ntiles, nclasses);
}

template <int MODE, int EPI = 0>
void launch_conv_tap(const bf16_t* a, const bf16_t* w, bf16_t* y, const ConvGeom& g,
                     hipStream_t st, float* slab = nullptr, const float* shift = nullptr,
                     const ConvBnEpi& ep = ConvBnEpi{}) {
  if (g.M == 0) return;
  const int nclasses = MODE == kDgrad3 || MODE == kDgrad1 ? 4 : 1;
  constexpr bool k1 = MODE == kFwd1 || MODE == kDgrad1;
  if (EPI == 1 && MODE == kFwd1 && g.NC % 128 == 0 && g.M >= 50176 && g.KC < 256) {
    const dim3 grid = conv_grid((g.M + 63) / 64, g.NC / 128, nclasses, k1);
    if (g_bnbwd_early && g.KC <= 128)
      hipLaunchKernelGGL((conv_tap_k<MODE, 64, 128, 2, 2, 3, EPI, kCT, 32, true>), grid, dim3(kCT), 0, st, a, w, y, g, slab, shift, ep);
    else
      hipLaunchKernelGGL((conv_tap_k<MODE, 64, 128, 2, 2, 3, EPI, kCT, 32>), grid, dim3(kCT), 0, st, a, w, y, g, slab, shift, ep);
  } else if (MODE == kFwd1 && g.NC % 128 == 0 && g.KC / kBK <= 1) {
    const dim3 grid = conv_grid((g.M + kBM - 1) / kBM, g.NC / 128, nclasses, k1);
    hipLaunchKernelGGL((conv_tap_k<MODE, 128, 128, 2, 2, 1, EPI>), grid, dim3(kCT), 0, st, a, w, y, g, slab, shift, ep);
  } else if (g.NC % 128 == 0) {
    const dim3 grid = conv_grid((g.M + kBM - 1) / kBM, g.NC / 128, nclasses, k1);
    if (grid.x * grid.y * grid.z >= 1024)
      hipLaunchKernelGGL((conv_tap_k<MODE, 128, 128, 2, 2, 3, EPI, kCT, 32>), grid, dim3(kCT), 0, st, a, w, y, g, slab, shift, ep);
    else
      hipLaunchKernelGGL((conv_tap_k<MODE, 128, 128, 2, 2, 2, EPI>), grid, dim3(kCT), 0, st, a, w, y, g, slab, shift, ep);
  } else {
    const dim3 grid = conv_grid((g.M + kBM - 1) / kBM, g.NC / 64, nclasses, k1);
    hipLaunchKernelGGL((conv_tap_k<MODE, 128, 64, 4, 1, 3, EPI, kCT, 32>), grid, dim3(kCT), 0, st, a, w, y, g, slab, shift, ep);
  }
}

constexpr int kHBM = 256;
constexpr int halo_rows(int BN) { return BN == 128 ? 448 : 512; }
constexpr uint32_t kHZero = 0x80000000u;

__device__ __forceinline__ int halo_ppos(int p, int H, int W, int HW) {
  const int n = p / HW, r = p - n * HW;
  const int h = r / W, w = r - h * W;
  return (n * (H + 2) + h + 1) * (W + 2) + w + 1;
}

__device__ __forceinline__ void buf_lds16(__amdgpu_buffer_rsrc_t r, unsigned char* dst,
                                          uint32_t voff, uint32_t soff) {
  __builtin_amdgcn_raw_ptr_buffer_load_lds(r, (__attribute__((address_space(3))) void*)dst, 16,
                                           voff, soff, 0, 0);
}

constexpr int conv3h_hcount(int t, int nhp) {
  return t < 0 || t >= 4 ? 0 : (nhp - 2 * t < 2 ? nhp - 2 * t : 2);
}

template <int N>
__device__ __forceinline__ void vm_wait_c() {
  asm volatile("s_waitcnt vmcnt(%0)" ::"n"(N) : "memory");
}

template <int BN, int EPI, int BM_ = kHBM>
__global__ void __launch_bounds__(kCT, 2)
    conv3h_k(const bf16_t* __restrict__ x, const bf16_t* __restrict__ wt,
             bf16_t* __restrict__ y, ConvGeom g, float* __restrict__ slab,
             const float* __restrict__ shift, ConvBnEpi ep) {
  constexpr int BM = BM_, CT = kCT, WM = BN == 128 ? 2 : 4, WN = 4 / WM;
  static_assert(BM % (16 * WM) == 0, "16-row fragments per wave");
  constexpr int kHRows = halo_rows(BN), kHBuf = kHRows * 64;
  constexpr int TM = BM / WM, TN = BN / WN, FM = TM / 16, FN = TN / 16;
  constexpr int BSLOT = BN * 64;
  constexpr int BPW = BN / 64;
  constexpr int NHP = kHRows / 64;
  constexpr int RING = 2 * kHBuf + 3 * BSLOT;
  constexpr int TS = BN + 8;
  constexpr int EPI_BYTES = BM * TS * 2;
  constexpr int LDS_BYTES = RING > EPI_BYTES ? RING : EPI_BYTES;
  static_assert(LDS_BYTES <= 80 * 1024, "two workgroups per CU");
  __shared__ __attribute__((aligned(1024))) unsigned char lds[LDS_BYTES];
  unsigned char* const hbuf = lds;
  unsigned char* const bring = lds + 2 * kHBuf;

  const int tid = threadIdx.x, lane = tid & 63;
  const int wid = __builtin_amdgcn_readfirstlane(tid >> 6);
  const int wm = wid / WN, wn = wid % WN;
  const int NTf = gridDim.y == 1 ? g.NC / BN : 1;
  const int lt = xcd_remap(blockIdx.x, gridDim.x);
  const int mt = lt / NTf, MTn = (int)gridDim.x / NTf;
  const int m0 = mt * BM, n0 = (gridDim.y == 1 ? lt - mt * NTf : (int)blockIdx.y) * BN;
  const int H = g.GH, W = g.GW, HW = H * W, Wp = W + 2, HpWp = (H + 2) * Wp;
  const int M = g.M, KC = g.KC;
  const int p1 = min(m0 + BM, M) - 1;
  const int base = halo_ppos(m0, H, W, HW) - Wp - 1;
  const int pend = halo_ppos(p1, H, W, HW) + Wp + 1;
  const int lrow = lane >> 2, pch = lane & 3;

  const int64_t pix0 = (int64_t)(base / HpWp) * HW;
  const __amdgpu_buffer_rsrc_t rx = __builtin_amdgcn_make_buffer_rsrc(
      const_cast<bf16_t*>(x + pix0 * KC), 0, 0x7fffffff, 0x00020000);
  uint32_t hoff[NHP];
#pragma unroll
  for (int u = 0; u < NHP; ++u) {
    const int row = (wid + 4 * u) * 16 + lrow;
    const int q = base + row;
    const int n = q / HpWp, rr = q - n * HpWp;
    const int hp = rr / Wp, wp = rr - hp * Wp;
    const bool ok = q <= pend && hp >= 1 && hp <= H && wp >= 1 && wp <= W;
    const int64_t pix = (int64_t)(n * H + hp - 1) * W + wp - 1 - pix0;
    hoff[u] = ok ? (uint32_t)(pix * KC * 2) + (uint32_t)((pch ^ swz_key<64>(row)) * 16) : kHZero;
  }
  const __amdgpu_buffer_rsrc_t rw = __builtin_amdgcn_make_buffer_rsrc(
      const_cast<bf16_t*>(wt + (int64_t)n0 * g.kb_stride), 0, 0x7fffffff, 0x00020000);
  uint32_t woff[BPW];
#pragma unroll
  for (int u = 0; u < BPW; ++u) {
    const int row = (wid * BPW + u) * 16 + lrow;
// ... 1018 lines not shown
                  const int* taps, int n, hipStream_t st) {
  for (int b = 0; b < n; b += kPrepMax) {
    PrepArgs a;
    std::memset(&a, 0, sizeof(a));
    a.n = n - b < kPrepMax ? n - b : kPrepMax;
    int tiles = 0;
    for (int i = 0; i < a.n; ++i) {
      const int k = b + i;
      a.d[i] = PrepDesc{static_cast<const uint16_t*>(w[k]), static_cast<uint16_t*>(out[k]),
                        cout[k], cin[k], taps[k], tiles};
      tiles += ((cout[k] + 63) / 64) * ((cin[k] + 63) / 64) * taps[k];
    }
    if (tiles > 0) hipLaunchKernelGGL(prep_weights_k, dim3(tiles), dim3(256), 0, st, a);
  }
}

void conv1x1_transpose_weight(const void* w, void* out, int Cout, int Cin, hipStream_t st) {
  hipLaunchKernelGGL(rot_weight_k, dim3((Cout + 63) / 64, (Cin + 63) / 64, 1), dim3(256), 0, st,
                     static_cast<const uint16_t*>(w), static_cast<uint16_t*>(out), Cout, Cin, 1);
}

void conv_halo_enable(int mode) { g_conv_halo = mode; }
void conv_halo_mtile(int bm) { g_conv_halo_bm = bm; }
void conv_bnbwd_early(int mode) { g_bnbwd_early = mode; }
int conv_halo_enabled() { return g_conv_halo; }

int g_conv1x1_g4w = 0;

bool conv1x1_g4w(int64_t M, int Cin, int Cout, int stride) {
  if (g_conv1x1_g4w == 0 || stride != 1 || Cout % 256 != 0 || Cin % 64 != 0 ||
      M >= ((int64_t)1 << 31) || !gemm4w_supported((int)M, Cout, Cin))
    return false;
  if (g_conv1x1_g4w == 2) return true;
  return (Cin == 512 && Cout == 2048) || (Cin == 1024 && Cout == 256) ||
         (Cin == 64 && Cout == 256);
}
void conv_1x1_gemm4w(int mode) { g_conv1x1_g4w = mode; }
void conv_nfast(int mode) { g_conv_nfast = mode; }
void conv_halo_nfast(int on) { g_conv3h_nfast = on; }
bool conv_1x1_on_gemm4w(int64_t M, int Cin, int Cout) { return conv1x1_g4w(M, Cin, Cout, 1); }

int conv_fwd_mtiles(int N, int H, int W, int Cout, int stride, int ksize, int Cin) {
  const int Ho = (H - 1) / stride + 1, Wo = (W - 1) / stride + 1;
  const int64_t M = (int64_t)N * Ho * Wo;
  if (ksize == 3 && conv3h_ok(N, H, W, Cout, stride)) {
    const int bm = conv3h_mtile(N, H, W, Cout);
    return (int)((M + bm - 1) / bm);
  }
  if (ksize == 1 && conv1x1_g4w(M, Cin, Cout, stride)) return (int)((M + 255) / 256);
  return (int)((M + kBM - 1) / kBM);
}

void conv_nhwc_fwd(const void* x, const void* w, void* y, int N, int H, int W, int Cin, int Cout,
                   int ksize, int stride, hipStream_t st, float* stats_slab,
                   const float* stats_shift) {
  const int Ho = (H - 1) / stride + 1, Wo = (W - 1) / stride + 1;
  const ConvGeom g{Ho, Wo, H, W, stride, Ho, Wo, 1, Cin, Cout, N * Ho * Wo, ksize * ksize * Cin};
  const auto* xp = static_cast<const bf16_t*>(x);
  const auto* wp = static_cast<const bf16_t*>(w);
  auto* yp = static_cast<bf16_t*>(y);
  if (ksize == 1 && conv1x1_g4w((int64_t)N * Ho * Wo, Cin, Cout, stride)) {
    GemmArgs a;
    std::memset(&a, 0, sizeof(a));
    a.A = x;
    a.B = w;
    a.C = y;
    a.M = N * Ho * Wo;
    a.N = Cout;
    a.K = Cin;
    a.lda = Cin;
    a.ldb = Cin;
    a.ldc = Cout;
    a.slab = stats_slab;
    a.shift = stats_shift;
    gemm4w(a, stats_slab ? 3 : 0, st);
    return;
  }
  if (ksize == 3 && conv3h_ok(N, H, W, Cout, stride))
    launch_conv3h<0>(xp, wp, yp, g, N, st, stats_slab, stats_shift, ConvBnEpi{});
  else if (ksize == 3) launch_conv_tap<kFwd3>(xp, wp, yp, g, st, stats_slab, stats_shift);
  else launch_conv_tap<kFwd1>(xp, wp, yp, g, st, stats_slab, stats_shift);
}

int conv_bnbwd_mtiles(int N, int H, int W, int Cout, int ksize, int Cin) {
  const int64_t M = (int64_t)N * H * W;
  if (ksize == 1 && Cout % 128 == 0 && M >= 50176 && Cin < 256) return (int)((M + 63) / 64);
  if (ksize == 3 && conv3h_ok(N, H, W, Cout, 1)) {
    const int bm = conv3h_mtile(N, H, W, Cout);
    return (int)((M + bm - 1) / bm);
  }
  return (int)((M + kBM - 1) / kBM);
}
void conv_nhwc_fwd_bnbwd(const void* dy, const void* w, void* gout, int N, int H, int W, int Cin,
                         int Cout, int ksize, int stride, const ConvBnEpi& ep, float* slab,
                         hipStream_t st) {
  const int Ho = (H - 1) / stride + 1, Wo = (W - 1) / stride + 1;
  const ConvGeom g{Ho, Wo, H, W, stride, Ho, Wo, 1, Cin, Cout, N * Ho * Wo, ksize * ksize * Cin};
  const auto* xp = static_cast<const bf16_t*>(dy);
  const auto* wp = static_cast<const bf16_t*>(w);
  auto* yp = static_cast<bf16_t*>(gout);
  if (ksize == 3 && stride == 1 && conv3h_ok(N, H, W, Cout, 1))
    launch_conv3h<1>(xp, wp, yp, g, N, st, slab, nullptr, ep);
  else if (ksize == 3) launch_conv_tap<kFwd3, 1>(xp, wp, yp, g, st, slab, nullptr, ep);
  else launch_conv_tap<kFwd1, 1>(xp, wp, yp, g, st, slab, nullptr, ep);
}

void conv_nhwc_dgrad_s2(const void* dy, const void* wt, void* dx, int N, int H, int W, int Cin,
                        int Cout, int ksize, hipStream_t st) {
  const int Ho = H / 2, Wo = W / 2;
  const ConvGeom g{Ho, Wo, Ho, Wo, 1, H, W, 2, Cout, Cin, N * Ho * Wo, ksize * ksize * Cout};
  const auto* dyp = static_cast<const bf16_t*>(dy);
  const auto* wp = static_cast<const bf16_t*>(wt);
  auto* dxp = static_cast<bf16_t*>(dx);
  if (ksize == 3) launch_conv_tap<kDgrad3>(dyp, wp, dxp, g, st);
  else launch_conv_tap<kDgrad1>(dyp, wp, dxp, g, st);
}

int conv_dgrad_s2_bnbwd_mtiles(int N, int H, int W) {
  const int64_t M = (int64_t)N * (H / 2) * (W / 2);
  return 4 * (int)((M + kBM - 1) / kBM);
}
void conv_nhwc_dgrad_s2_bnbwd(const void* dy, const void* wt, void* gout, int N, int H, int W,
                              int Cin, int Cout, const ConvBnEpi& ep, float* slab,
                              hipStream_t st) {
  const int Ho = H / 2, Wo = W / 2;
  const ConvGeom g{Ho, Wo, Ho, Wo, 1, H, W, 2, Cout, Cin, N * Ho * Wo, 9 * Cout};
  launch_conv_tap<kDgrad3, 1>(static_cast<const bf16_t*>(dy), static_cast<const bf16_t*>(wt),
                              static_cast<bf16_t*>(gout), g, st, slab, nullptr, ep);
}

}
```

csrc/include/amd_kernels.h:

```cpp
#pragma once
#include <hip/hip_runtime.h>
#include <stdint.h>
#include "mt_table.h"

namespace amd {

enum class DType : int;

struct ScaleArg {
  const float* ptr;
  float val;
  int invert;
};

void mt_scale(const MTLaunch& L, DType in, DType out, ScaleArg s, int* noop, hipStream_t st);
void mt_check_finite(const MTLaunch& L, DType in, int* noop, hipStream_t st);
void mt_axpby(const MTLaunch& L, DType x, DType y, DType out, ScaleArg a, ScaleArg b,
              int arg_to_check, int* noop, hipStream_t st);
void mt_fill_zero(const MTLaunch& L, DType t, hipStream_t st);
void mt_copy_if(const MTLaunch& L, DType t, const int* flag, hipStream_t st);

void mt_norm_partials(const MTLaunch& L, DType in, int max_norm, float* partials, int* noop,
                      hipStream_t st);
void mt_norm_finalize(const MTLaunch& L, const float* partials, int npart_sets, int max_norm,
// ... 152 lines not shown
                    const float* invstd, const void* weight, const void* bias, DType tw,
                    int relu, const void* z, const uint8_t* relu_mask, int64_t outer, int64_t C,
                    int64_t inner,
                    int channel_last, float* sum_dy, float* sum_dy_xmu, void* grad_weight,
                    void* grad_bias, float* ws, hipStream_t st,
                    const float* sum_scale = nullptr);
void bn_backward_elemt(const void* dy, const void* x, DType tx, const float* mean,
                       const float* invstd, const void* weight, const void* bias, DType tw,
                       const float* sum_dy, const float* sum_dy_xmu, float inv_count,
                       int relu, const void* z, const uint8_t* relu_mask, void* dx, void* dz,
                       int64_t outer, int64_t C, int64_t inner, int channel_last, hipStream_t st);


void maxpool2d_nhwc_fwd(const void* x, DType t, void* y, uint8_t* idx, int N, int H, int W, int C,
                        int OH, int OW, int k, int s, int p, hipStream_t st,
                        const float* mean = nullptr, const float* invstd = nullptr,
                        const float* bw = nullptr, const float* bb = nullptr);
void maxpool2d_nhwc_bwd(const void* dy, const uint8_t* idx, DType t, void* dx, int N, int H,
                        int W, int C, int OH, int OW, int k, int s, int p, hipStream_t st);
bool maxpool2d_nhwc_bwd_bn_ok(int H, int W, int C, int OH, int OW, int k, int s, int p);
int maxpool_bwd_bn_grid(int N, int H, int W);
void maxpool2d_nhwc_bwd_bn(const void* dy, const uint8_t* idx, DType t, void* dx, int N, int H,
                           int W, int C, int OH, int OW, const void* x, const float* mean,
                           const float* invstd, const float* bw, const float* bb, float* slab,
                           hipStream_t st);
void gap_nhwc_bwd(const void* dy, DType t, void* dx, int64_t N, int64_t HW, int C,
                  hipStream_t st);

struct GemmArgs {
  const void* A;
  const void* B;
  void* C;
  int M, N, K, lda, ldb, ldc;
  const void* bias;
  int bias_f32;
  void* aux;
  float* colsum;
  int tanh;
  int fp16;
  int group_m;
  float* slab;
  const float* shift;
};
bool gemm4w_supported(int M, int N, int K);
void gemm4w(const GemmArgs& a, int epi, hipStream_t st);
struct WgradArgs {
  const void* A;
  const void* B;
  float* P;
  int M, N, lda, ldb;
  int rows;
  int S;
  int fp16;
  int group_m;
  float* colsum = nullptr;
};
bool wgrad4w_supported(int64_t T, int M, int N, int S);
void wgrad4w(const WgradArgs& a, hipStream_t st);

bool conv3x3_nhwc_supported(int Cin, int Cout);
void conv_halo_enable(int mode);
void conv_nfast(int mode);
void conv_halo_nfast(int on);
void conv_halo_mtile(int bm);
int conv_halo_enabled();
void conv_bnbwd_early(int mode);
void conv_1x1_gemm4w(int mode);
bool conv_1x1_on_gemm4w(int64_t M, int Cin, int Cout);
void conv_nhwc_fwd(const void* x, const void* w, void* y, int N, int H, int W, int Cin, int Cout,
                   int ksize, int stride, hipStream_t st, float* stats_slab = nullptr,
                   const float* stats_shift = nullptr);
int conv_fwd_mtiles(int N, int H, int W, int Cout, int stride, int ksize, int Cin);
int conv_bnbwd_mtiles(int N, int H, int W, int Cout, int ksize, int Cin);
struct ConvBnEpi {
  const void* add;
  const void* xbn;
  const uint8_t* rmask;
  const float* mean;
  const float* invstd;
  const float* w;
  const float* b;
  int relu_mode;
  int add_s2;
};
void conv_nhwc_fwd_bnbwd(const void* dy, const void* w, void* g, int N, int H, int W, int Cin,
                         int Cout, int ksize, int stride, const ConvBnEpi& ep, float* slab,
                         hipStream_t st);
void bn_slab_train_stats(const float* slab, int S, int64_t C, int64_t count, const float* shift,
                         float* mean, float* invstd, float* running_mean, float* running_var,
                         long long* nbt, float eps, float momentum, hipStream_t st);
void bn_slab_packed_stats(const float* slab, int S, int64_t C, int64_t count, const float* shift,
                          float* packed, hipStream_t st);
bool bn_grad_accumulate();
void bn_set_grad_accumulate(bool on);
struct BNAccumScope {
  bool prev;
  explicit BNAccumScope(bool on) : prev(bn_grad_accumulate()) { bn_set_grad_accumulate(on); }
  ~BNAccumScope() { bn_set_grad_accumulate(prev); }
};
void bn_slab_reduce_grad(const float* slab, int S, int64_t C, const float* invstd,
                         float* sum_dy, float* sum_dy_xmu, void* gw, void* gb, DType tw,
                         hipStream_t st, const float* sum_scale = nullptr);
void conv_nhwc_dgrad_s2(const void* dy, const void* wt, void* dx, int N, int H, int W, int Cin,
                        int Cout, int ksize, hipStream_t st);
int conv_dgrad_s2_bnbwd_mtiles(int N, int H, int W);
void conv_nhwc_dgrad_s2_bnbwd(const void* dy, const void* wt, void* gout, int N, int H, int W,
                              int Cin, int Cout, const ConvBnEpi& ep, float* slab,
                              hipStream_t st);
int conv_wgrad_splits(int N, int H, int W, int Cin, int Cout, int ksize, int stride, int algo);
bool conv3x3_wgrad_supported(int W, int algo);
bool conv3x3_wgrad_c64_ok(int W, int Cin, int Cout, int ksize, int stride);
int64_t conv_wgrad_workspace(int S, int Cin, int Cout, int ksize);
int64_t splitk_reduce_workspace(int S, int64_t n);
void splitk_reduce(const float* part, int S, int Cout, int Cin, float* stage, void* out,
                   bool out_fp32, hipStream_t st, bool accum = false);
void conv3x3_rot_weight(const void* w, void* out, int Cout, int Cin, hipStream_t st);
void conv1x1_transpose_weight(const void* w, void* out, int Cout, int Cin, hipStream_t st);
void prep_weights(const void* const* w, void* const* out, const int* cout, const int* cin,
                  const int* taps, int n, hipStream_t st);
void conv_nhwc_wgrad(const void* dy, const void* x, float* part, void* dw, bool dw_fp32, int N,
                     int H, int W, int Cin, int Cout, int ksize, int stride, int S, int algo,
                     hipStream_t st, bool accum = false);

bool stem_conv_supported(int N, int H, int W);
void stem_pad(const void* x, void* xp, int N, int H, int W, hipStream_t st);
void stem_fwd(const void* xp, const void* wk, void* y, int N, int H, int W, hipStream_t st,
              float* slab = nullptr, const float* shift = nullptr);
int stem_fwd_slab_width(int N, int H);
int stem_wgrad_splits(int N, int H);
void stem_wgrad(const void* xp, const void* dy, float* part, int S, int N, int H, int W,
                hipStream_t st);

int colsum_splits(int64_t M, int N);
void colsum_finalize(const float* part, int S, int N, void* out, DType tb, hipStream_t st);
void gelu_fwd(const void* x, void* y, DType t, int64_t n, bool tanh_approx, hipStream_t st);
void colsum(const void* x, const void* pre, void* out_dpre, DType t, int64_t M, int N,
            int act_mode, float* part, int S, void* bias_grad, DType tb, hipStream_t st);

struct AttnView {
  void* p = nullptr;
  int64_t sb = 0, ss = 0, sh = 0;
};
struct AttnProblem {
  AttnView q, k, v;
  int B, H;
  int Sq, Sk;
  float scale, dropout;
  uint32_t seed;
  bool causal;
  DType dtype;
  const float* kbias = nullptr;
  const unsigned char* klive = nullptr;
};
int attn_lse_stride(int S);
void attn_fwd(const AttnProblem& p, void* o, float* lse, hipStream_t st);

enum class AttnMaskKind : int { Bool8 = 0, F32 = 1, F16 = 2, BF16 = 3 };
void attn_prepare_key_mask(const void* mask, AttnMaskKind kind, int B, int S, float* bias,
                           unsigned char* live, hipStream_t st);

struct AttnBwd {
  AttnView o, dout;
  AttnView dq, dk, dv;
  const float* lse;
  float* D;
};
void attn_bwd(const AttnProblem& p, const AttnBwd& g, hipStream_t st);

void xentropy_fwd(const void* x, DType tx, const int64_t* labels, int64_t rows, int V,
                  float smoothing, int64_t padding_idx, void* loss, DType tloss, float* lse,
// ... 12 lines not shown
```

csrc/include/bn_common.h:

```cpp
#pragma once
#include "amd_dev.h"
#include "amd_kernels.h"

#include <type_traits>

namespace amd {

constexpr int kBNThreads = 256;

template <typename F>
static inline void bn_dispatch(DType a, F&& f) {
  switch (a) {
    case DType::F32: f(float{}); break;
    case DType::F16: f(half_t{}); break;
    case DType::BF16: f(bf16_t{}); break;
    default: break;
  }
}

static inline bool all_aligned(std::initializer_list<const void*> ps) {
  for (const void* p : ps)
    if (p && ((uintptr_t)p % 16) != 0) return false;
  return true;
}

__device__ __forceinline__ void chan_affine(const float* mean, const float* invstd, float w,
                                            float b, int c, float& sc, float& sh) {
  float is = invstd[c];
  sc = is * w;
  sh = b - mean[c] * sc;
}

template <typename TW>
__device__ __forceinline__ float wload(const TW* p, int c, float dflt) {
  return p ? to_f32(p[c]) : dflt;
}

template <int CH>
__device__ __forceinline__ void slab_sum(const float* __restrict__ slab, int splits, int C, int c0,
                                         float* out ) {
  __shared__ float red[kBNThreads / kWave][2 * CH];
  float a[2 * CH];
#pragma unroll
  for (int k = 0; k < 2 * CH; ++k) a[k] = 0.f;
  for (int s = threadIdx.x; s < splits; s += blockDim.x) {
    const float* row = slab + (size_t)s * 2 * C;
#pragma unroll
    for (int k = 0; k < CH; ++k) {
      if (c0 + k < C) {
        a[k] += row[c0 + k];
        a[CH + k] += row[C + c0 + k];
      }
    }
  }
  const int lane = threadIdx.x & (kWave - 1), wid = threadIdx.x / kWave;
#pragma unroll
  for (int k = 0; k < 2 * CH; ++k) a[k] = wave_sum(a[k]);
  if (lane == 0) {
#pragma unroll
    for (int k = 0; k < 2 * CH; ++k) red[wid][k] = a[k];
  }
  __syncthreads();
  if (threadIdx.x < 2 * CH) {
    float t = 0.f;
    for (int w = 0; w < (int)(blockDim.x / kWave); ++w) t += red[w][threadIdx.x];
    out[threadIdx.x] = t;
  }
  __syncthreads();
}

struct BNStatsOut {
  float* mean;
  float* var;
  float* invstd;
  float* running_mean;
  float* running_var;
  long long* nbt;
  float eps, momentum;
  float* count_out = nullptr;
  float count_val = 0.f;
};

template <typename T, int CH>
__global__ void __launch_bounds__(kBNThreads)
    stats_finalize(const T* __restrict__ x, const float* __restrict__ slab, int splits, int C,
                   int64_t count, int64_t shift_stride, BNStatsOut out) {
  __shared__ float sums[2 * CH];
  const int c0 = blockIdx.x * CH;
  slab_sum<CH>(slab, splits, C, c0, sums);
  const int k = threadIdx.x;
  if (k < CH && c0 + k < C) {
    const int c = c0 + k;
    const float shift = to_f32(x[(int64_t)c * shift_stride]);
    double m = (double)sums[k] / (double)count;
    double v = (double)sums[CH + k] / (double)count - m * m;
    if (v < 0.0) v = 0.0;
    const float mean = (float)(shift + m);
    out.mean[c] = mean;
    if (out.var) out.var[c] = (float)v;
    if (out.invstd) out.invstd[c] = rsqrtf((float)v + out.eps);
    if (out.running_mean) {
      const double unb = count > 1 ? v * (double)count / (double)(count - 1) : v;
      out.running_mean[c] = (1.f - out.momentum) * out.running_mean[c] + out.momentum * mean;
      out.running_var[c] = (1.f - out.momentum) * out.running_var[c] + out.momentum * (float)unb;
    }
    if (out.nbt && c == 0) *out.nbt += 1;
    if (out.count_out && c == 0) *out.count_out = out.count_val;
  }
}

template <typename TW, int CH>
__global__ void __launch_bounds__(kBNThreads)
    reduce_finalize(const float* __restrict__ slab, int splits, int C,
// ... 81 lines not shown
```

csrc/torch/module.cpp:

```cpp
#include <torch/extension.h>

#include "amd_kernels.h"
#include "amp_ops.h"
#include "attn_ops.h"
#include "norm_ops.h"
#include "pool_ops.h"
#include "dense_ops.h"
#include "lt_ops.h"
#include "xent_ops.h"
#include "emb_ops.h"
#include "reducer.h"

#include <hip/hip_runtime_api.h>

#include <cstdint>
#include <vector>

namespace py = pybind11;
using namespace amd;

static at::Tensor flatten_dense(const std::vector<at::Tensor>& ts) {
  std::vector<at::Tensor> flat;
  flat.reserve(ts.size());
  for (auto& t : ts) flat.push_back(t.contiguous().view({-1}));
// ... 43 lines not shown
  mt.def("advance_step", &advance_step_op);
  mt.def("mark_step_done", &mark_step_done_op);
  mt.def("flat_scale", &flat_scale_op);
  py::class_<StepPlan, std::shared_ptr<StepPlan>>(mt, "StepPlan")
      .def(py::init<std::vector<at::Tensor>, TensorLists>(), py::arg("owners"), py::arg("fixed"))
      .def("refresh", &StepPlan::refresh)
      .def("set_absent", &StepPlan::set_absent)
      .def("sgd", &StepPlan::sgd)
      .def("sgd_pair", &StepPlan::sgd_pair)
      .def("adam", &StepPlan::adam)
      .def("grad_norm_into", &StepPlan::grad_norm_into)
      .def("lamb", &StepPlan::lamb)
      .def("size", &StepPlan::size)
      .def("rebuilds", &StepPlan::rebuilds);
  mt.def("plan_cache_clear", &mt_plan_cache_clear);
  mt.def("plan_cache_size", &mt_plan_cache_size);

  auto ac = m.def_submodule("apex_C", "flatten / unflatten (apex_C parity)");
  ac.def("flatten", &flatten_dense);
  ac.def("unflatten", &unflatten_dense);

  auto ln = m.def_submodule("layer_norm", "fused LayerNorm / RMSNorm (wave64 row kernels)");
  ln.def("forward", &layer_norm_forward_op);
  ln.def("backward", &layer_norm_backward_op);
  ln.def("add_dropout_forward", &add_dropout_layer_norm_forward_op);
  ln.def("add_dropout_backward", &add_dropout_layer_norm_backward_op);
  ln.def("set_bwd_one_row", &layer_norm_bwd_one_row);
  ln.def("bwd_one_row", &layer_norm_bwd_one_row_on);

  auto attn = m.def_submodule("attn", "fused attention (head dim 64, MFMA, gfx950)");
  attn.def("fwd", &attn_fwd_op, py::arg("q"), py::arg("k"), py::arg("v"), py::arg("causal"),
           py::arg("dropout"), py::arg("seed"), py::arg("scale"),
           py::arg("key_bias") = py::none(), py::arg("key_live") = py::none());
  attn.def("bwd", &attn_bwd_op, py::arg("dout"), py::arg("q"), py::arg("k"), py::arg("v"),
           py::arg("o"), py::arg("lse"), py::arg("causal"), py::arg("dropout"), py::arg("seed"),
           py::arg("scale"), py::arg("dq"), py::arg("dk"), py::arg("dv"),
           py::arg("key_bias") = py::none(), py::arg("key_live") = py::none());
  attn.def("prepare_key_mask", &attn_prepare_key_mask_op, py::arg("mask"), py::arg("S"));

  auto dn = m.def_submodule("dense", "dense-layer bias gradients / fused GELU backward");
  dn.def("bias_grad", &bias_grad_op);
  dn.def("gelu_bwd_bias_grad", &gelu_bwd_bias_grad_op);
  dn.def("act_bwd_bias_grad", &act_bwd_bias_grad_op);
  dn.def("gelu", &gelu_fwd_op);
  dn.def("gelu_fwd_lt", &dense_gelu_fwd_op);
  dn.def("dgelu_bgrad_lt", &dense_dgelu_bgrad_op);
  dn.def("lt_cache_clear", &lt_algo_cache_clear);
  dn.def("lt_probe", &lt_probe_op);
  dn.def("wgrad_bgrad_lt", &dense_wgrad_bgrad_op);
  dn.def("gemm4w", &gemm4w_op, py::arg("a"), py::arg("b"), py::arg("epi") = 0,
         py::arg("bias") = py::none(), py::arg("aux") = py::none(), py::arg("want_pre") = false,
         py::arg("tanh") = false, py::arg("bias_grad_dtype") = py::none());
  dn.def("gemm4w_ok", &gemm4w_ok);
  dn.def("wgrad4w", &wgrad4w_op, py::arg("dy"), py::arg("x"), py::arg("splits"),
         py::arg("out_dtype"), py::arg("out") = py::none(), py::arg("accumulate") = true);
  dn.def("wgrad4w_ok", &wgrad4w_ok);
  dn.def("wgrad4w_bias", &wgrad4w_bias_op, py::arg("dy"), py::arg("x"), py::arg("splits"),
         py::arg("out_dtype"), py::arg("out") = py::none(), py::arg("accumulate") = true,
         py::arg("bias_dtype") = at::kFloat);
  auto xe = m.def_submodule("xentropy", "fused softmax cross entropy + label smoothing");
  xe.def("forward", &xentropy_fwd_op);
  xe.def("backward", &xentropy_bwd_op);

  auto emb = m.def_submodule("emb", "deterministic embedding weight gradient (no host sync)");
  emb.def("wgrad", &embedding_wgrad_op, py::arg("idx"), py::arg("dy"), py::arg("V"),
          py::arg("padding_idx"), py::arg("out_dtype"));

  auto pool = m.def_submodule("pool", "NHWC max pooling (gather backward, no atomics)");
  pool.def("max_fwd", &maxpool2d_nhwc_fwd_op);
  pool.def("max_bwd", &maxpool2d_nhwc_bwd_op);
  pool.def("max_bwd_bn", &maxpool2d_nhwc_bwd_bn_op, py::arg("dy"), py::arg("idx"), py::arg("H"),
           py::arg("W"), py::arg("x"), py::arg("mean"), py::arg("invstd"),
           py::arg("weight") = py::none(), py::arg("bias") = py::none());
  pool.def("gap_bwd", &gap_nhwc_bwd_op, py::arg("dy"), py::arg("H"), py::arg("W"));
  pool.def("max_fwd_bn", &maxpool2d_nhwc_bn_fwd_op);
  auto conv = m.def_submodule("conv", "MFMA implicit-GEMM convolutions (NHWC bf16)");
  conv.def("conv_fwd", &conv_nhwc_fwd_op, py::arg("x"), py::arg("w"), py::arg("stride") = 1);
  conv.def("conv_fwd_bnbwd", &conv_nhwc_fwd_bnbwd_op, py::arg("dy"), py::arg("w"),
           py::arg("add"), py::arg("x"), py::arg("rmask"), py::arg("mean"), py::arg("invstd"),
           py::arg("bn_weight"), py::arg("bn_bias"), py::arg("relu_mode"),
           py::arg("add_stride2") = false);
  conv.def("conv_fwd_stats", &conv_nhwc_fwd_stats_op, py::arg("x"), py::arg("w"),
           py::arg("stride") = 1, py::arg("shift") = py::none());
  conv.def("conv_dgrad_s2", &conv_nhwc_dgrad_s2_op);
  conv.def("conv_dgrad_s2_bnbwd", &conv_nhwc_dgrad_s2_bnbwd_op, py::arg("dy"), py::arg("wt"),
           py::arg("H"), py::arg("W"), py::arg("x"), py::arg("rmask"), py::arg("mean"),
           py::arg("invstd"), py::arg("bn_weight"), py::arg("bn_bias"), py::arg("relu_mode"));
  conv.def("conv_wgrad", &conv_nhwc_wgrad_op, py::arg("dy"), py::arg("x"), py::arg("out_dtype"),
           py::arg("algo") = 0, py::arg("stride") = 1, py::arg("ksize") = 3,
           py::arg("out") = py::none(), py::arg("accumulate") = true);
  conv.def("splitk_reduce", &splitk_reduce_op, py::arg("part"), py::arg("out_dtype"),
           py::arg("out") = py::none(), py::arg("accumulate") = true);
  conv.def("stem_pad", &stem_pad_op);
  conv.def("stem_fwd", &stem_fwd_op);
  conv.def("stem_fwd_stats", &stem_fwd_stats_op, py::arg("xp"), py::arg("wk"),
           py::arg("shift") = py::none());
  conv.def("stem_wgrad", &stem_wgrad_op);
  conv.def("rot_weight", &conv3x3_rot_weight_op);
  conv.def("transpose_weight", &conv1x1_transpose_weight_op);
  conv.def("prep_weights", &conv_prep_weights_op);
  conv.def("set_nfast", &conv_nfast, py::arg("mode"));
  conv.def("set_halo_nfast", &conv_halo_nfast, py::arg("on"));
  conv.def("set_halo", &conv_halo_enable, py::arg("mode"),
           "3x3 stride-1 convs on the halo-resident kernel: 0 off, 1 auto, 64 / 128 force "
           "that output-tile width where possible");
  conv.def("halo_enabled", &conv_halo_enabled);
  conv.def("set_halo_mtile", &conv_halo_mtile, py::arg("bm"));
  conv.def("set_bnbwd_early", &conv_bnbwd_early);
  conv.def("set_1x1_gemm4w", &conv_1x1_gemm4w);
  conv.def("on_gemm4w_1x1", &conv_1x1_on_gemm4w, py::arg("M"), py::arg("Cin"), py::arg("Cout"));

  auto bn = m.def_submodule("bn", "BatchNorm / SyncBatchNorm kernels (NCHW + NHWC)");
  bn.def("local_stats", &bn_local_stats_op);
  bn.def("train_stats", &bn_train_stats_op);
  bn.def("combine_stats", &bn_combine_stats_op);
  bn.def("apply", &bn_apply_op);
  bn.def("forward_local", &bn_forward_local_op, py::arg("x"), py::arg("weight"),
         py::arg("bias"), py::arg("running_mean"), py::arg("running_var"), py::arg("nbt"),
         py::arg("eps"), py::arg("momentum"), py::arg("z"), py::arg("relu"),
         py::arg("want_mask") = false);
  bn.def("apply_mask", &bn_apply_mask_op);
  bn.def("slab_train_stats", &bn_slab_train_stats_op, py::arg("slab"), py::arg("count"),
         py::arg("shift"), py::arg("running_mean"), py::arg("running_var"), py::arg("nbt"),
         py::arg("eps"), py::arg("momentum"));
  bn.def("slab_reduce_grad", &bn_slab_reduce_grad_op, py::arg("slab"), py::arg("invstd"),
         py::arg("weight"), py::arg("need_wgrad"), py::arg("sum_scale") = py::none(),
         py::arg("grad_weight") = py::none(), py::arg("grad_bias") = py::none(),
         py::arg("accumulate") = true);
  bn.def("slab_packed_stats", &bn_slab_packed_stats_op, py::arg("slab"), py::arg("count"),
         py::arg("shift"), py::arg("out") = py::none());
  bn.def("set_tuning", &bn_set_tuning, py::arg("red_rpt") = -1, py::arg("red_cap") = -1,
         py::arg("red_min") = -1, py::arg("elem_rpt") = -1, py::arg("elem_cap") = -1,
         py::arg("elem_min") = -1);
  bn.def("get_tuning", []() {
    int o[6];
    bn_get_tuning(o);
    return std::vector<int>(o, o + 6);
  });
  bn.def("reduce_grad", &bn_reduce_grad_op, py::arg("dy"), py::arg("x"), py::arg("mean"),
         py::arg("invstd"), py::arg("weight"), py::arg("bias"), py::arg("z"), py::arg("relu"),
         py::arg("need_wgrad"), py::arg("mask") = py::none(),
         py::arg("sum_scale") = py::none(), py::arg("grad_weight") = py::none(),
         py::arg("grad_bias") = py::none(), py::arg("accumulate") = true);
  bn.def("local_stats_packed", &bn_local_stats_packed_op, py::arg("x"),
         py::arg("out") = py::none());
  bn.def("combine_stats_sync", &bn_combine_stats_sync_op, py::arg("gathered"), py::arg("eps"),
         py::arg("momentum"), py::arg("running_mean"), py::arg("running_var"),
         py::arg("nbt") = py::none());
  bn.def("backward_elemt", &bn_backward_elemt_op, py::arg("dy"), py::arg("x"), py::arg("mean"),
         py::arg("invstd"), py::arg("weight"), py::arg("bias"), py::arg("sum_dy"),
         py::arg("sum_dy_xmu"), py::arg("count"), py::arg("z"), py::arg("relu"),
         py::arg("want_dz"), py::arg("mask") = py::none());

  bn.def("backward_x2_ok", &bn_backward_x2_ok);
  bn.def("apply2_mask", &bn_apply2_mask_op, py::arg("x"), py::arg("mean"), py::arg("invstd"),
         py::arg("weight"), py::arg("bias"), py::arg("xz"), py::arg("meanz"), py::arg("invstdz"),
         py::arg("weightz"), py::arg("biasz"));
  bn.def("backward_elemt_x2", &bn_backward_elemt_x2_op, py::arg("dy"), py::arg("x"),
         py::arg("mean"), py::arg("invstd"), py::arg("weight"), py::arg("bias"),
         py::arg("sum_dy"), py::arg("sum_dy_xmu"), py::arg("count"), py::arg("x2"),
         py::arg("mean2"), py::arg("invstd2"), py::arg("weight2"), py::arg("need_wgrad2"));
  bn.def("backward_local", &bn_backward_local_op, py::arg("dy"), py::arg("x"), py::arg("mean"),
         py::arg("invstd"), py::arg("weight"), py::arg("bias"), py::arg("z"), py::arg("relu"),
         py::arg("need_wgrad"), py::arg("want_dz"), py::arg("mask") = py::none());

  auto rd = m.def_submodule("reducer", "DDP bucketed gradient reducer core");
// ... 3 lines not shown
```

csrc/torch/pool_ops.cpp:

```cpp
#include <cstdlib>
#include "pool_ops.h"

#include "common.h"

namespace amd {

namespace {
int64_t out_size(int64_t in, int64_t k, int64_t s, int64_t p) { return (in + 2 * p - k) / s + 1; }
}

std::tuple<at::Tensor, at::Tensor> maxpool2d_nhwc_fwd_op(at::Tensor x, int64_t k, int64_t s,
                                                         int64_t p) {
  return maxpool2d_nhwc_bn_fwd_op(x, c10::nullopt, c10::nullopt, c10::nullopt, c10::nullopt, k, s,
                                  p);
}

std::tuple<at::Tensor, at::Tensor> maxpool2d_nhwc_bn_fwd_op(
    at::Tensor x, c10::optional<at::Tensor> mean, c10::optional<at::Tensor> invstd,
    c10::optional<at::Tensor> w, c10::optional<at::Tensor> b, int64_t k, int64_t s, int64_t p) {
  c10::NoGradGuard no_grad_;
  auto f32 = [&](const c10::optional<at::Tensor>& t) -> const float* {
    if (!t.has_value() || !t->defined()) return nullptr;
    TORCH_CHECK(t->scalar_type() == at::kFloat && t->is_contiguous() && t->is_cuda() &&
                    t->numel() == x.size(1),
// ... 57 lines not shown
  const float* mp = f32c(mean, "mean");
  const float* ip = f32c(invstd, "invstd");
  const float* wp = weight.has_value() && weight->defined() ? f32c(*weight, "weight") : nullptr;
  const float* bp = bias.has_value() && bias->defined() ? f32c(*bias, "bias") : nullptr;
  at::Tensor dx = at::empty({N, C, H, W}, dy.options().memory_format(at::MemoryFormat::ChannelsLast));
  at::Tensor slab = at::empty({2, C, (int64_t)maxpool_bwd_bn_grid((int)N, (int)H, (int)W)},
                              dy.options().dtype(at::kFloat));
  TORCH_CHECK((uintptr_t)dy.data_ptr() % 16 == 0 && (uintptr_t)dx.data_ptr() % 16 == 0 &&
                  (uintptr_t)x.data_ptr() % 16 == 0 && (uintptr_t)idx.data_ptr() % 8 == 0,
              "max_bwd_bn: 16-byte aligned tensors expected");
  maxpool2d_nhwc_bwd_bn(dy.data_ptr(), idx.data_ptr<uint8_t>(), dtype_of(dy), dx.data_ptr(),
                        (int)N, (int)H, (int)W, (int)C, (int)OH, (int)OW, x.data_ptr(), mp, ip,
                        wp, bp, slab.data_ptr<float>(), cur_stream());
  return {dx, slab};
}

at::Tensor gap_nhwc_bwd_op(at::Tensor dy, int64_t H, int64_t W) {
  c10::NoGradGuard no_grad_;
  TORCH_CHECK(dy.is_cuda() && (dy.dim() == 2 || dy.dim() == 4), "gap_bwd: dy [N, C(, 1, 1)]");
  const int64_t N = dy.size(0), C = dy.size(1);
  TORCH_CHECK(dy.numel() == N * C, "gap_bwd: dy must hold one value per (n, c)");
  dy = dy.reshape({N, C}).contiguous();
  at::Tensor dx =
      at::empty({N, C, H, W}, dy.options().memory_format(at::MemoryFormat::ChannelsLast));
  gap_nhwc_bwd(dy.data_ptr(), dtype_of(dy), dx.data_ptr(), N, H * W, (int)C, cur_stream());
  return dx;
}

}

namespace amd {

at::Tensor conv_nhwc_fwd_op(at::Tensor x, at::Tensor w, int64_t stride) {
  c10::NoGradGuard no_grad_;
  TORCH_CHECK(x.is_cuda() && x.dim() == 4 && w.dim() == 4, "conv: 4-D GPU tensors expected");
  TORCH_CHECK(x.scalar_type() == at::kBFloat16 && w.scalar_type() == at::kBFloat16,
              "conv: bf16 only");
  TORCH_CHECK(stride == 1 || stride == 2, "conv: stride 1 or 2");
  const int64_t N = x.size(0), Cin = x.size(1), H = x.size(2), W = x.size(3);
  const int64_t Cout = w.size(0), k = w.size(2);
  TORCH_CHECK((k == 3 || k == 1) && w.size(3) == k && w.size(1) == Cin, "conv: weight shape");
  const int64_t Ho = (H - 1) / stride + 1, Wo = (W - 1) / stride + 1;
  TORCH_CHECK(conv3x3_nhwc_supported((int)Cin, (int)Cout), "conv: channels must be x64");
  TORCH_CHECK(N * H * W < (int64_t)1 << 31, "conv: too many pixels");
  x = x.contiguous(at::MemoryFormat::ChannelsLast);
  w = w.contiguous(at::MemoryFormat::ChannelsLast);
  at::Tensor y = at::empty({N, Cout, Ho, Wo},
                           x.options().memory_format(at::MemoryFormat::ChannelsLast));
  conv_nhwc_fwd(x.data_ptr(), w.data_ptr(), y.data_ptr(), (int)N, (int)H, (int)W, (int)Cin,
                (int)Cout, (int)k, (int)stride, cur_stream());
  return y;
}

std::tuple<at::Tensor, at::Tensor> conv_nhwc_fwd_stats_op(at::Tensor x, at::Tensor w,
                                                          int64_t stride,
                                                          c10::optional<at::Tensor> shift) {
  c10::NoGradGuard no_grad_;
  TORCH_CHECK(x.is_cuda() && x.dim() == 4 && w.dim() == 4, "conv: 4-D GPU tensors expected");
  TORCH_CHECK(x.scalar_type() == at::kBFloat16 && w.scalar_type() == at::kBFloat16,
              "conv: bf16 only");
  TORCH_CHECK(stride == 1 || stride == 2, "conv: stride 1 or 2");
  const int64_t N = x.size(0), Cin = x.size(1), H = x.size(2), W = x.size(3);
  const int64_t Cout = w.size(0), k = w.size(2);
  TORCH_CHECK((k == 3 || k == 1) && w.size(3) == k && w.size(1) == Cin, "conv: weight shape");
  const int64_t Ho = (H - 1) / stride + 1, Wo = (W - 1) / stride + 1;
  TORCH_CHECK(conv3x3_nhwc_supported((int)Cin, (int)Cout), "conv: channels must be x64");
  TORCH_CHECK(N * H * W < (int64_t)1 << 31, "conv: too many pixels");
  const float* sp = nullptr;
  if (shift.has_value() && shift->defined()) {
    TORCH_CHECK(shift->scalar_type() == at::kFloat && shift->is_contiguous() &&
                    shift->numel() == Cout && shift->is_cuda(),
                "conv stats: shift must be a contiguous fp32 [Cout] GPU tensor");
    sp = shift->data_ptr<float>();
  }
  x = x.contiguous(at::MemoryFormat::ChannelsLast);
  w = w.contiguous(at::MemoryFormat::ChannelsLast);
  at::Tensor y = at::empty({N, Cout, Ho, Wo},
                           x.options().memory_format(at::MemoryFormat::ChannelsLast));
  const int S = conv_fwd_mtiles((int)N, (int)H, (int)W, (int)Cout, (int)stride, (int)k, (int)Cin);
  at::Tensor slab = at::empty({2, Cout, S}, x.options().dtype(at::kFloat));
  conv_nhwc_fwd(x.data_ptr(), w.data_ptr(), y.data_ptr(), (int)N, (int)H, (int)W, (int)Cin,
                (int)Cout, (int)k, (int)stride, cur_stream(), slab.data_ptr<float>(), sp);
  return {y, slab};
}

std::tuple<at::Tensor, at::Tensor> conv_nhwc_fwd_bnbwd_op(
    at::Tensor dy, at::Tensor w, c10::optional<at::Tensor> add, at::Tensor xbn,
    c10::optional<at::Tensor> rmask, at::Tensor mean, at::Tensor invstd,
    c10::optional<at::Tensor> bn_w, c10::optional<at::Tensor> bn_b, int64_t relu_mode,
    bool add_stride2) {
  c10::NoGradGuard no_grad_;
  TORCH_CHECK(dy.is_cuda() && dy.dim() == 4 && w.dim() == 4, "conv_bnbwd: 4-D GPU tensors");
  TORCH_CHECK(dy.scalar_type() == at::kBFloat16 && w.scalar_type() == at::kBFloat16 &&
                  xbn.scalar_type() == at::kBFloat16,
              "conv_bnbwd: bf16 only");
  const int64_t N = dy.size(0), Cin = dy.size(1), H = dy.size(2), W = dy.size(3);
  const int64_t Cout = w.size(0), k = w.size(2);
  TORCH_CHECK((k == 3 || k == 1) && w.size(3) == k && w.size(1) == Cin, "conv_bnbwd: weight");
  TORCH_CHECK(conv3x3_nhwc_supported((int)Cin, (int)Cout), "conv_bnbwd: channels must be x64");
  TORCH_CHECK(N * H * W < (int64_t)1 << 31, "conv_bnbwd: too many pixels");
  TORCH_CHECK(relu_mode >= 0 && relu_mode <= 2, "conv_bnbwd: relu_mode 0 | 1 | 2");
  const auto cl = at::MemoryFormat::ChannelsLast;
  auto same_out = [&](const at::Tensor& t, const char* what) {
    TORCH_CHECK(t.is_cuda() && t.dim() == 4 && t.size(0) == N && t.size(1) == Cout &&
                    t.size(2) == H && t.size(3) == W && t.scalar_type() == at::kBFloat16 &&
                    t.is_contiguous(cl),
                "conv_bnbwd: ", what, " must be a channels-last bf16 tensor shaped like the output");
  };
  same_out(xbn, "x");
  ConvBnEpi ep{};
  if (add.has_value() && add->defined()) {
    if (add_stride2) {
      TORCH_CHECK(k == 1 && H % 2 == 0 && W % 2 == 0 && add->is_cuda() && add->dim() == 4 &&
                      add->size(0) == N && add->size(1) == Cout && add->size(2) == H / 2 &&
                      add->size(3) == W / 2 && add->scalar_type() == at::kBFloat16 &&
                      add->is_contiguous(cl),
                  "conv_bnbwd: a stride-2 add must be channels-last bf16 [N, C, H/2, W/2] "
                  "(1x1 conv, even H and W)");
      ep.add_s2 = 1;
    } else {
      same_out(*add, "add");
    }
    ep.add = add->data_ptr();
  }
  ep.xbn = xbn.data_ptr();
  auto vecf = [&](const c10::optional<at::Tensor>& t, const char* what) -> const float* {
    if (!t.has_value() || !t->defined()) return nullptr;
    TORCH_CHECK(t->is_cuda() && t->scalar_type() == at::kFloat && t->is_contiguous() &&
                    t->numel() == Cout,
                "conv_bnbwd: ", what, " must be a contiguous fp32 [C] GPU tensor");
    return t->data_ptr<float>();
  };
  ep.mean = vecf(mean, "mean");
  ep.invstd = vecf(invstd, "invstd");
  ep.w = vecf(bn_w, "weight");
  ep.b = vecf(bn_b, "bias");
  TORCH_CHECK(ep.mean && ep.invstd, "conv_bnbwd: mean / invstd required");
  ep.relu_mode = (int)relu_mode;
  if (relu_mode == 1) {
    TORCH_CHECK(rmask.has_value() && rmask->defined() && rmask->is_cuda() &&
                    rmask->scalar_type() == at::kByte && rmask->is_contiguous() &&
                    rmask->numel() == N * H * W * (Cout / 8),
                "conv_bnbwd: relu_mode 1 needs the forward's [M][C/8] uint8 bitmask");
    ep.rmask = rmask->data_ptr<uint8_t>();
  }
  dy = dy.contiguous(cl);
  w = w.contiguous(cl);
  at::Tensor g = at::empty({N, Cout, H, W}, dy.options().memory_format(cl));
  const int S = conv_bnbwd_mtiles((int)N, (int)H, (int)W, (int)Cout, (int)k, (int)Cin);
  at::Tensor slab = at::empty({2, Cout, S}, dy.options().dtype(at::kFloat));
  conv_nhwc_fwd_bnbwd(dy.data_ptr(), w.data_ptr(), g.data_ptr(), (int)N, (int)H, (int)W,
                      (int)Cin, (int)Cout, (int)k, 1, ep, slab.data_ptr<float>(), cur_stream());
  return {g, slab};
}

at::Tensor conv_nhwc_dgrad_s2_op(at::Tensor dy, at::Tensor wt, int64_t H, int64_t W) {
  c10::NoGradGuard no_grad_;
  TORCH_CHECK(dy.is_cuda() && dy.dim() == 4 && wt.dim() == 4, "conv_dgrad_s2: 4-D GPU tensors");
  TORCH_CHECK(dy.scalar_type() == at::kBFloat16 && wt.scalar_type() == at::kBFloat16,
              "conv_dgrad_s2: bf16 only");
  const int64_t N = dy.size(0), Cout = dy.size(1), Ho = dy.size(2), Wo = dy.size(3);
  const int64_t Cin = wt.size(0), k = wt.size(2);
  TORCH_CHECK(wt.size(1) == Cout && (k == 3 || k == 1) && wt.size(3) == k,
              "conv_dgrad_s2: transposed / rotated weight [Cin, Cout, k, k] expected");
  TORCH_CHECK(H == 2 * Ho && W == 2 * Wo, "conv_dgrad_s2: even input sizes only");
  TORCH_CHECK(conv3x3_nhwc_supported((int)Cout, (int)Cin), "conv_dgrad_s2: channels x64");
// ... 254 lines not shown
```

csrc/torch/pool_ops.h:

```cpp
#pragma once
#include <ATen/ATen.h>
#include <c10/util/Optional.h>

#include <tuple>

namespace amd {

std::tuple<at::Tensor, at::Tensor> maxpool2d_nhwc_fwd_op(at::Tensor x, int64_t k, int64_t s,
                                                         int64_t p);
std::tuple<at::Tensor, at::Tensor> maxpool2d_nhwc_bn_fwd_op(
    at::Tensor x, c10::optional<at::Tensor> mean, c10::optional<at::Tensor> invstd,
    c10::optional<at::Tensor> w, c10::optional<at::Tensor> b, int64_t k, int64_t s, int64_t p);
at::Tensor maxpool2d_nhwc_bwd_op(at::Tensor dy, at::Tensor idx, int64_t H, int64_t W, int64_t k,
                                 int64_t s, int64_t p);
at::Tensor gap_nhwc_bwd_op(at::Tensor dy, int64_t H, int64_t W);

at::Tensor conv_nhwc_fwd_op(at::Tensor x, at::Tensor w, int64_t stride);
std::tuple<at::Tensor, at::Tensor> conv_nhwc_fwd_stats_op(at::Tensor x, at::Tensor w,
                                                          int64_t stride,
                                                          c10::optional<at::Tensor> shift);
std::tuple<at::Tensor, at::Tensor> conv_nhwc_fwd_bnbwd_op(
    at::Tensor dy, at::Tensor w, c10::optional<at::Tensor> add, at::Tensor xbn,
    c10::optional<at::Tensor> rmask, at::Tensor mean, at::Tensor invstd,
    c10::optional<at::Tensor> bn_w, c10::optional<at::Tensor> bn_b, int64_t relu_mode,
    bool add_stride2 = false);
at::Tensor conv_nhwc_dgrad_s2_op(at::Tensor dy, at::Tensor wt, int64_t H, int64_t W);
at::Tensor conv_nhwc_wgrad_op(at::Tensor dy, at::Tensor x, at::ScalarType out_dtype, int64_t algo,
                              int64_t stride, int64_t ksize, c10::optional<at::Tensor> out, bool accumulate = true);
at::Tensor splitk_reduce_op(at::Tensor part, at::ScalarType out_dtype,
                            c10::optional<at::Tensor> out_acc, bool accumulate = true);
at::Tensor stem_pad_op(at::Tensor x);
at::Tensor stem_fwd_op(at::Tensor xp, at::Tensor wk);
std::tuple<at::Tensor, at::Tensor> conv_nhwc_dgrad_s2_bnbwd_op(
    at::Tensor dy, at::Tensor wt, int64_t H, int64_t W, at::Tensor xbn,
    c10::optional<at::Tensor> rmask, at::Tensor mean, at::Tensor invstd,
    c10::optional<at::Tensor> bn_w, c10::optional<at::Tensor> bn_b, int64_t relu_mode);
std::tuple<at::Tensor, at::Tensor> maxpool2d_nhwc_bwd_bn_op(at::Tensor dy, at::Tensor idx,
                                                            int64_t H, int64_t W, at::Tensor x,
                                                            at::Tensor mean, at::Tensor invstd,
                                                            c10::optional<at::Tensor> weight,
                                                            c10::optional<at::Tensor> bias);
std::tuple<at::Tensor, at::Tensor> stem_fwd_stats_op(at::Tensor xp, at::Tensor wk,
                                                     c10::optional<at::Tensor> shift);
at::Tensor stem_wgrad_op(at::Tensor xp, at::Tensor dy);
at::Tensor conv3x3_rot_weight_op(at::Tensor w);
at::Tensor conv1x1_transpose_weight_op(at::Tensor w);
std::vector<at::Tensor> conv_prep_weights_op(std::vector<at::Tensor> ws);

}
```

Baseline: 12730 images/s.

## Recompute bottleneck conv3 output inside fused BN apply and BN backward epilogues

For non-downsample bottleneck blocks with selected channel shapes, conv3 now runs a stats-only pass whose output is never written, then recomputes the 1x1 GEMM inside a fused kernel that applies BN, adds the residual, applies ReLU and writes the mask. In backward it recomputes the conv output again inside the BN backward-elementwise epilogue rather than reading the saved activation. This trades extra GEMM FLOPs for fewer reads and writes of the large 256- and 512-channel activations, and adds matching-logic state passed through thread-local storage and tensor attributes.

```diff
diff --git a/apex_example_amd/models/resnet.py b/apex_example_amd/models/resnet.py
--- a/apex_example_amd/models/resnet.py
+++ b/apex_example_amd/models/resnet.py
@@ -114,6 +114,8 @@
         out = self.bn2(self.conv2(out))
         if proj is not None and fuse_ds:
             return bn_add_bn_relu(self.bn3.bn, self.conv3(out), self.downsample.bn.bn, proj)
+        if self.downsample is None and self.bn3.fused and isinstance(self.conv3, Conv2d1x1):
+            return self.bn3(self.conv3.forward_bn3(out, identity), identity)
         return self.bn3(self.conv3(out), identity)
 
 
diff --git a/apex_example_amd/ops/batch_norm.py b/apex_example_amd/ops/batch_norm.py
--- a/apex_example_amd/ops/batch_norm.py
+++ b/apex_example_amd/ops/batch_norm.py
@@ -33,6 +33,27 @@
         self.x, self.mean, self.invstd = x, mean, invstd
         self.weight, self.bias, self.mask, self.relu_mode = weight, bias, mask, relu_mode
         self.result = None
+
+
+class ConvRec:
+    __slots__ = ("a", "w", "bwd", "applied")
+
+    def __init__(self, a, w, bwd):
+        self.a, self.w, self.bwd = a, w, bwd
+        self.applied = None
+
+    def take_applied(self, z, weight, bias):
+        ent, self.applied = self.applied, None
+        if ent is None or z is None or weight is None or bias is None:
+            return None
+        if (ent[0].data_ptr() != z.data_ptr() or ent[0].shape != z.shape
+                or ent[1] is not weight or ent[2] is not bias):
+            return None
+        return ent[3], ent[4]
+
+
+REC_FWD_CALLS = [0]
+REC_BWD_CALLS = [0]
 
 
 def _bwd_src(x, xl, mean, invstd, weight, bias, mask, fuse_relu, has_z):
@@ -195,12 +216,19 @@
             world = dist.get_world_size(process_group)
         collective = world > 1 or bool(force_collectives)
         want_mask = bool(fuse_relu) and zl is not None and xl.is_cuda
+        rec, _TLS.rec = getattr(_TLS, "rec", None), None
+        ctx.rec = None
         if not collective and xl.is_cuda:
             if slab is not None:
                 mean_g, invstd = C.slab_train_stats(slab, count, slab_shift, running_mean,
                                                     running_var, num_batches_tracked,
                                                     float(eps), float(momentum))
-                if want_mask:
+                done = (rec.take_applied(zl, weight, bias)
+                        if rec is not None and want_mask and x is xl else None)
+                if done is not None:
+                    REC_FWD_CALLS[0] += 1
+                    y, mask = done
+                elif want_mask:
                     y, mask = C.apply_mask(xl, mean_g, invstd, weight, bias, zl, bool(fuse_relu))
                 else:
                     y, mask = C.apply(xl, mean_g, invstd, weight, bias, zl, bool(fuse_relu)), None
@@ -218,6 +246,8 @@
             zg = getattr(z, "grad_fn", None) if z is not None else None
             ctx.zctx = zg if isinstance(zg, BatchNormFunction._backward_cls) else None
             ctx.pre = None
+            if rec is not None and rec.bwd and x is xl and weight is not None:
+                ctx.rec = rec
             ctx.orig_shape, ctx.has_z, ctx.shape_channel_last = orig_shape, z is not None, \
                 shape_channel_last
             return y.view(orig_shape) if shape_channel_last else y
@@ -335,8 +365,14 @@
                     zc.pre = (dyl.data_ptr(), dyl._version, s1, s2, gw2, gb2)
                     return (dx, dyl, gw if need_w else None, gb if need_w else None, None, None,
                             None, None, None, None, None, None, None, None, None)
-            dx, _ = C.backward_elemt(dyl, xl, mean, invstd, weight, bias, sum_dy, sum_dy_xmu,
-                                     total, None, False, False)
+            rec, ctx.rec = ctx.rec, None
+            if rec is not None and ctx.world == 1:
+                REC_BWD_CALLS[0] += 1
+                dx = _native.require().conv.conv1x1_bn_bwd(
+                    rec.a, rec.w, dyl, mean, invstd, weight, sum_dy, sum_dy_xmu, total)
+            else:
+                dx, _ = C.backward_elemt(dyl, xl, mean, invstd, weight, bias, sum_dy,
+                                         sum_dy_xmu, total, None, False, False)
             return (dx, dyl if ctx.has_z else None, gw if need_w else None,
                     gb if need_w else None, None, None, None, None, None, None, None, None, None,
                     None, None)
@@ -415,9 +451,11 @@
 
 def batch_norm_act(x, weight, bias, running_mean, running_var, training, momentum, eps,
                    z=None, fuse_relu=False, process_group=False, shape_channel_last=False,
-                   num_batches_tracked=None, force_collectives=False, slab=None, slab_shift=None):
+                   num_batches_tracked=None, force_collectives=False, slab=None, slab_shift=None,
+                   rec=None):
     if training:
         _TLS.src = None
+        _TLS.rec = rec
         y = BatchNormFunction.apply(x, z, weight, bias, running_mean, running_var, eps, momentum,
                                     process_group, fuse_relu, shape_channel_last,
                                     num_batches_tracked, force_collectives, slab, slab_shift)
@@ -451,6 +489,7 @@
 
     def forward(self, x, z=None):
         slab, shift = take_slab(x, self)
+        rec = x.__dict__.pop("_amd_bn_rec", None) if isinstance(x, torch.Tensor) else None
         if not x.is_cuda and not _native.available():
             y = super().forward(x)
             if z is not None:
@@ -470,7 +509,7 @@
                               self.running_var if self.track_running_stats else None,
                               use_batch, momentum, self.eps, z=z, fuse_relu=self.fuse_relu,
                               process_group=False, num_batches_tracked=nbt,
-                              slab=slab if use_batch else None, slab_shift=shift)
+                              slab=slab if use_batch else None, slab_shift=shift, rec=rec)
 
 
 _FUSE_DS = os.environ.get("APEX_AMD_BN_DS_FUSE", "1") == "1"
diff --git a/apex_example_amd/ops/conv.py b/apex_example_amd/ops/conv.py
--- a/apex_example_amd/ops/conv.py
+++ b/apex_example_amd/ops/conv.py
@@ -10,7 +10,7 @@
 
 from .. import _native
 from . import _ddp_direct
-from .batch_norm import bn_src_of
+from .batch_norm import BatchNorm2dReLU, ConvRec, bn_src_of
 
 _USE_WSTREAM = os.environ.get("APEX_AMD_WGRAD_STREAM", "1") == "1"
 _SIDE = {}
@@ -319,9 +319,50 @@
     return g
 
 
+_BN3_RECOMPUTE = True
+_REC_FWD = {(64, 256)}
+_REC_BWD = {(64, 256), (128, 512)}
+
+
+def _recompute_plan(conv, x, z):
+    ci, co = conv.in_channels, conv.out_channels
+    fwd, bwd = (ci, co) in _REC_FWD, (ci, co) in _REC_BWD
+    if not (_BN3_RECOMPUTE and (fwd or bwd) and conv._gemm_ok(x) and x.dtype == torch.bfloat16
+            and ci % 64 == 0 and ci <= 128 and co % 128 == 0 and _native.available()):
+        return None, None
+    bn = _stats_bn(conv, x)
+    n, _, h, w = x.shape
+    if not (type(bn) is BatchNorm2dReLU and bn.fuse_relu and bn.affine
+            and bn.track_running_stats and bn.momentum is not None
+            and bn.weight.dtype == torch.float32 and bn.bias.dtype == torch.float32
+            and bn.weight.is_contiguous() and bn.bias.is_contiguous()
+            and _shift_of(bn) is not None and bn.running_var.dtype == torch.float32
+            and isinstance(z, torch.Tensor) and z.is_cuda and z.dtype == torch.bfloat16
+            and tuple(z.shape) == (n, co, h, w)
+            and z.is_contiguous(memory_format=torch.channels_last)
+            and z.data_ptr() % 16 == 0):
+        return None, None
+    import torch.distributed as dist
+    if dist.is_available() and dist.is_initialized() and dist.get_world_size() > 1:
+        return None, None
+    if not _native.require().conv.recompute_1x1_ok(n * h * w, ci, co):
+        return None, None
+    return ConvRec(x.detach(), conv.weight.detach(), bwd), bn if fwd else None
+
+
+def _apply_now(rec, bn, x3, z):
+    C = _native.require()
+    slab, shift, _ = x3._amd_bn_stats
+    count = x3.numel() // x3.size(1)
+    mean, invstd = C.bn.slab_train_stats(slab, count, shift, None, None, None, float(bn.eps),
+                                         0.0)
+    y, mask = C.conv.conv1x1_bn_apply(rec.a, rec.w, x3, mean, invstd, bn.weight, bn.bias, z)
+    rec.applied = (z, bn.weight, bn.bias, y, mask)
+
+
 class Conv1x1GemmFunction(torch.autograd.Function):
     @staticmethod
-    def forward(ctx, x, weight, bn=None, src=None):
+    def forward(ctx, x, weight, bn=None, src=None, stats_only=False):
         ctx.save_for_backward(x, weight)
         ctx.src = src
         if ctx.needs_input_grad[1]:
@@ -330,6 +371,11 @@
         if ctx.needs_input_grad[0] and weight.dtype == torch.bfloat16 and (
                 src is not None or _own_1x1(x.dtype, weight.shape[0], ci, n * h * w)):
             _register_prep(weight)
+        if stats_only:
+            shift = _shift_of(bn)
+            y, slab = _native.require().conv.conv1x1_stats_only(x, weight, shift)
+            _TLS.slab = (slab, shift, bn)
+            return y
         return _conv1x1_fwd(x, weight, bn)
 
     @staticmethod
@@ -353,7 +399,7 @@
             else:
                 so, sa = _side_out(side, weight)
                 dw = side.run(lambda: _wgrad_1x1_w(dy, x, weight, so, sa), dy, x)
-        return dx, dw, None, None
+        return dx, dw, None, None, None
 
 
 class Conv1x1SkipFunction(torch.autograd.Function):
@@ -546,6 +592,17 @@
         return F.conv2d(x, self.weight, self.bias, self.stride, self.padding, self.dilation,
                         self.groups)
 
+    def forward_bn3(self, x, z):
+        rec, bn = _recompute_plan(self, x, z)
+        if rec is None:
+            return self.forward(x)
+        y = _tag_stats(Conv1x1GemmFunction.apply(x, self.weight, _stats_bn(self, x),
+                                                 bn_src_of(x), bn is not None))
+        if bn is not None:
+            _apply_now(rec, bn, y, z)
+        y._amd_bn_rec = rec
+        return y
+
     def forward_with_skip(self, x):
         if self._gemm_ok(x):
             y, skip = Conv1x1SkipFunction.apply(x, self.weight, _stats_bn(self, x),
diff --git a/csrc/hip/bn_nhwc.hip b/csrc/hip/bn_nhwc.hip
--- a/csrc/hip/bn_nhwc.hip
+++ b/csrc/hip/bn_nhwc.hip
@@ -238,11 +238,14 @@
       uint32_t mb = 0;
 #pragma unroll
       for (int i = 0; i < W; ++i) {
-        float o = fmaf(v[u][i], sc[i], sh[i]);
+        float o;
         if constexpr (ZA) {
+          o = fmaf(v[u][i], sc[i], sh[i]);
           o += to_f32(from_f32<T>(fmaf(zz[u][i], scz[i], shz[i])));
         } else if constexpr (ZZ) {
-          o += zz[u][i];
+          o = bn_apply_z(v[u][i], sc[i], sh[i], zz[u][i]);
+        } else {
+          o = fmaf(v[u][i], sc[i], sh[i]);
         }
         mb |= (o > 0.f ? 1u : 0u) << i;
         v[u][i] = relu ? fmaxf(o, 0.f) : o;
@@ -342,12 +345,8 @@
   stage_params(C, cb, ctile * W, [&](int c, int k) {
     const float wc = wload(w, c, 1.f);
     chan_affine(mean, invstd, wc, wload(b, c, 0.f), c, s_par[0][k], s_par[1][k]);
-    const float is = invstd[c];
-    const float mdy = sum_dy[c] * inv_n, mdyx = sum_dy_xmu[c] * inv_n;
-    const float q1 = is * wc, q2 = -is * is * is * wc * mdyx;
-    s_par[2][k] = q1;
-    s_par[3][k] = q2;
-    s_par[4][k] = -is * wc * mdy - q2 * mean[c];
+    bn_bwd_consts(invstd[c], wc, mean[c], sum_dy[c], sum_dy_xmu[c], inv_n, s_par[2][k],
+                  s_par[3][k], s_par[4][k]);
     if constexpr (X2) s_par[X2 ? 5 : 0][k] = mean2[c];
   });
   float t1[W], t2[W], m2[W];
@@ -397,7 +396,7 @@
           d = o > 0.f ? d : 0.f;
         }
         dv[u][i] = d;
-        xv[u][i] = fmaf(d, k1[i], fmaf(xv[u][i], k2[i], k3[i]));
+        xv[u][i] = bn_bwd_elem(d, xv[u][i], k1[i], k2[i], k3[i]);
         if constexpr (X2) {
           t1[i] += d;
           t2[i] = fmaf(d, x2v[u][i] - m2[i], t2[i]);
diff --git a/csrc/hip/conv_igemm.hip b/csrc/hip/conv_igemm.hip
--- a/csrc/hip/conv_igemm.hip
+++ b/csrc/hip/conv_igemm.hip
@@ -5,6 +5,7 @@
 
 #include "amd_dev.h"
 #include "amd_kernels.h"
+#include "bn_common.h"
 
 namespace amd {
 
@@ -235,10 +236,113 @@
   }
 }
 
+template <int BM, int BN, int CT = kCT>
+struct RecPre {
+  static constexpr int CPR = BN / 8;
+  static constexpr int RGS = CT / CPR;
+  static constexpr int ROWS = BM / RGS;
+  uint4 av[ROWS];
+  float mu[8], iv[8], wv[8], bv[8], sd[8], sx[8];
+};
+
+template <int EPI, int BM, int BN, int CT>
+__device__ __forceinline__ void rec_prefetch(const ConvGeom& g, const ConvBnEpi& ep, int m0,
+                                             int n0, RecPre<BM, BN, CT>& P) {
+  using PT = RecPre<BM, BN, CT>;
+  const int tid = threadIdx.x;
+  const int cc = tid % PT::CPR, rg = tid / PT::CPR;
+  const int c0 = n0 + cc * 8;
+  const float* zf = reinterpret_cast<const float*>(g_zero16);
+  {
+    const float* wp = ep.w ? ep.w + c0 : g_one8;
+    const float* bp = ep.b ? ep.b + c0 : zf;
+    const float* mp = ep.mean + c0;
+    const float* ip = ep.invstd + c0;
+    const float* dp = EPI == 4 ? ep.sum_dy + c0 : zf;
+    const float* xp = EPI == 4 ? ep.sum_dy_xmu + c0 : zf;
+#pragma unroll
+    for (int i = 0; i < 8; ++i) {
+      P.mu[i] = mp[i];
+      P.iv[i] = ip[i];
+      P.wv[i] = wp[i];
+      P.bv[i] = bp[i];
+      P.sd[i] = dp[i];
+      P.sx[i] = xp[i];
+    }
+  }
+  const bf16_t* addp = static_cast<const bf16_t*>(ep.add);
+#pragma unroll
+  for (int q = 0; q < PT::ROWS; ++q) {
+    const int m = m0 + q * PT::RGS + rg;
+    const int mm = m < g.M ? m : 0;
+    P.av[q] = *reinterpret_cast<const uint4*>(addp + (int64_t)mm * g.NC + c0);
+  }
+}
+
+template <int EPI, int BM, int BN, int CT, int TS>
+__device__ __forceinline__ void rec_store(const bf16_t* T, bf16_t* __restrict__ y,
+                                          const ConvGeom& g, const ConvBnEpi& ep, int m0, int n0,
+                                          const RecPre<BM, BN, CT>& P) {
+  using PT = RecPre<BM, BN, CT>;
+  const int tid = threadIdx.x;
+  const int cc = tid % PT::CPR, rg = tid / PT::CPR;
+  const int c0 = n0 + cc * 8;
+  __builtin_amdgcn_s_waitcnt(0x0F70);
+  float k1[8], k2[8], k3[8];
+#pragma unroll
+  for (int i = 0; i < 8; ++i) {
+    if constexpr (EPI == 3) {
+      chan_affine(P.mu, P.iv, P.wv[i], P.bv[i], i, k1[i], k2[i]);
+      k3[i] = 0.f;
+    } else {
+      bn_bwd_consts(P.iv[i], P.wv[i], P.mu[i], P.sd[i], P.sx[i], ep.inv_n, k1[i], k2[i], k3[i]);
+    }
+  }
+  bf16_t* y2 = static_cast<bf16_t*>(ep.out2);
+#pragma unroll
+  for (int q = 0; q < PT::ROWS; ++q) {
+    const int row = q * PT::RGS + rg;
+    const int m = m0 + row;
+    if (m >= g.M) continue;
+    const uint4 tv = *reinterpret_cast<const uint4*>(T + row * TS + cc * 8);
+    const int64_t off = (int64_t)m * g.NC + c0;
+    if constexpr (EPI == 3) *reinterpret_cast<uint4*>(y + off) = tv;
+    const unsigned tw[4] = {tv.x, tv.y, tv.z, tv.w};
+    const unsigned aw[4] = {P.av[q].x, P.av[q].y, P.av[q].z, P.av[q].w};
+    unsigned ow[4], mb = 0;
+#pragma unroll
+    for (int k = 0; k < 4; ++k) {
+      const float xx[2] = {__uint_as_float(tw[k] << 16), __uint_as_float(tw[k] & 0xffff0000u)};
+      const float aa[2] = {__uint_as_float(aw[k] << 16), __uint_as_float(aw[k] & 0xffff0000u)};
+      unsigned short hb[2];
+#pragma unroll
+      for (int h = 0; h < 2; ++h) {
+        const int i = 2 * k + h;
+        float r;
+        if constexpr (EPI == 3) {
+          const float o = bn_apply_z(xx[h], k1[i], k2[i], aa[h]);
+          mb |= (o > 0.f ? 1u : 0u) << i;
+          r = fmaxf(o, 0.f);
+        } else {
+          r = bn_bwd_elem(aa[h], xx[h], k1[i], k2[i], k3[i]);
+        }
+        hb[h] = __builtin_bit_cast(unsigned short, (bf16_t)r);
+      }
+      ow[k] = (unsigned)hb[0] | ((unsigned)hb[1] << 16);
+    }
+    if constexpr (EPI == 3) {
+      *reinterpret_cast<uint4*>(y2 + off) = make_uint4(ow[0], ow[1], ow[2], ow[3]);
+      ep.rmask_out[(int64_t)m * (g.NC >> 3) + (c0 >> 3)] = (uint8_t)mb;
+    } else {
+      *reinterpret_cast<uint4*>(y + off) = make_uint4(ow[0], ow[1], ow[2], ow[3]);
+    }
+  }
+}
+
 template <int MODE, int BM, int BN, int WM, int WN, int NB, int EPI = 0, int CT = kCT,
           int BK = kBK, bool EARLY = false>
 __global__ void __launch_bounds__(CT, (NB * (BM + BN) * BK * 2 > 80 * 1024)
-                                          ? 1 : (NB == 1 && EPI == 0 ? 3 : 2))
+                                          ? 1 : (NB == 1 && (EPI == 0 || EPI == 2) ? 3 : 2))
     conv_tap_k(const bf16_t* __restrict__ x, const bf16_t* __restrict__ wt,
                bf16_t* __restrict__ y, ConvGeom g, float* __restrict__ slab,
                const float* __restrict__ shift, ConvBnEpi ep) {
@@ -333,15 +437,17 @@
 
   const int fr = lane & 15, fg = lane >> 4;
   constexpr int CPR = BN / 8;
-  const bool want_stats = EPI == 1 ? slab != nullptr
+  constexpr bool plain = EPI == 0 || EPI == 2;
+  const bool want_stats = EPI >= 3 ? false : EPI == 1 ? slab != nullptr
                                    : (MODE == kFwd3 || MODE == kFwd1) && slab != nullptr;
   const int scc = tid % CPR;
   float shv[8];
 #pragma unroll
   for (int i = 0; i < 8; ++i)
-    shv[i] = (EPI == 0 && want_stats && shift) ? shift[n0 + scc * 8 + i] : 0.f;
+    shv[i] = (plain && want_stats && shift) ? shift[n0 + scc * 8 + i] : 0.f;
 
   BnPre<BM, BN, CT> pre;
+  RecPre<BM, BN, CT> rpre;
   if constexpr (EPI == 1 && EARLY) bnbwd_prefetch<MODE, BM, BN, CT>(g, ep, m0, n0, z, pre);
 
   {
@@ -389,6 +495,10 @@
   if constexpr (EPI == 1) {
     if constexpr (!EARLY) bnbwd_prefetch<MODE, BM, BN, CT>(g, ep, m0, n0, z, pre);
     lds_barrier();
+  } else if constexpr (EPI >= 3) {
+    static_assert(EPI < 3 || MODE == kFwd1, "recompute epilogues: dense 1x1 forward only");
+    rec_prefetch<EPI, BM, BN, CT>(g, ep, m0, n0, rpre);
+    lds_barrier();
   } else {
     __syncthreads();
   }
@@ -406,7 +516,7 @@
                           ((unsigned)__builtin_bit_cast(unsigned short, (bf16_t)acc[i][j][3]) << 16);
       *reinterpret_cast<uint2*>(T + row * TS + col) = make_uint2(lo, hi);
     }
-  if constexpr (EPI == 1) {
+  if constexpr (EPI == 1 || EPI >= 3) {
     lds_barrier();
   } else {
     __syncthreads();
@@ -417,6 +527,8 @@
   for (int i = 0; i < 8; ++i) s1[i] = s2[i] = 0.f;
   if constexpr (EPI == 1) {
     bnbwd_store<MODE, BM, BN, CT, TS>(T, y, g, ep, m0, n0, z, pre, s1, s2);
+  } else if constexpr (EPI >= 3) {
+    rec_store<EPI, BM, BN, CT, TS>(T, y, g, ep, m0, n0, rpre);
   } else
   for (int c = tid; c < BM * CPR; c += CT) {
     const int row = c / CPR, cc = c - row * CPR;
@@ -430,7 +542,7 @@
       opix = (int64_t)(n * g.YH + gh * g.ys + (z >> 1)) * g.YW + gw * g.ys + (z & 1);
     }
     const uint4 v = *reinterpret_cast<const uint4*>(T + row * TS + cc * 8);
-    *reinterpret_cast<uint4*>(y + opix * g.NC + n0 + cc * 8) = v;
+    if constexpr (EPI != 2) *reinterpret_cast<uint4*>(y + opix * g.NC + n0 + cc * 8) = v;
     if (want_stats) {
       const unsigned wv[4] = {v.x, v.y, v.z, v.w};
 #pragma unroll
@@ -488,13 +600,17 @@
   if (g.M == 0) return;
   const int nclasses = MODE == kDgrad3 || MODE == kDgrad1 ? 4 : 1;
   constexpr bool k1 = MODE == kFwd1 || MODE == kDgrad1;
-  if (EPI == 1 && MODE == kFwd1 && g.NC % 128 == 0 && g.M >= 50176 && g.KC < 256) {
-    const dim3 grid = conv_grid((g.M + 63) / 64, g.NC / 128, nclasses, k1);
-    if (g_bnbwd_early && g.KC <= 128)
-      hipLaunchKernelGGL((conv_tap_k<MODE, 64, 128, 2, 2, 3, EPI, kCT, 32, true>), grid, dim3(kCT), 0, st, a, w, y, g, slab, shift, ep);
-    else
-      hipLaunchKernelGGL((conv_tap_k<MODE, 64, 128, 2, 2, 3, EPI, kCT, 32>), grid, dim3(kCT), 0, st, a, w, y, g, slab, shift, ep);
-  } else if (MODE == kFwd1 && g.NC % 128 == 0 && g.KC / kBK <= 1) {
+  if constexpr (EPI == 1 && MODE == kFwd1) {
+    if (g.NC % 128 == 0 && g.M >= 50176 && g.KC < 256) {
+      const dim3 grid = conv_grid((g.M + 63) / 64, g.NC / 128, nclasses, k1);
+      if (g_bnbwd_early && g.KC <= 128)
+        hipLaunchKernelGGL((conv_tap_k<MODE, 64, 128, 2, 2, 3, EPI, kCT, 32, true>), grid, dim3(kCT), 0, st, a, w, y, g, slab, shift, ep);
+      else
+        hipLaunchKernelGGL((conv_tap_k<MODE, 64, 128, 2, 2, 3, EPI, kCT, 32>), grid, dim3(kCT), 0, st, a, w, y, g, slab, shift, ep);
+      return;
+    }
+  }
+  if (MODE == kFwd1 && g.NC % 128 == 0 && g.KC / kBK <= 1) {
     const dim3 grid = conv_grid((g.M + kBM - 1) / kBM, g.NC / 128, nclasses, k1);
     hipLaunchKernelGGL((conv_tap_k<MODE, 128, 128, 2, 2, 1, EPI>), grid, dim3(kCT), 0, st, a, w, y, g, slab, shift, ep);
   } else if (g.NC % 128 == 0) {
@@ -503,9 +619,11 @@
       hipLaunchKernelGGL((conv_tap_k<MODE, 128, 128, 2, 2, 3, EPI, kCT, 32>), grid, dim3(kCT), 0, st, a, w, y, g, slab, shift, ep);
     else
       hipLaunchKernelGGL((conv_tap_k<MODE, 128, 128, 2, 2, 2, EPI>), grid, dim3(kCT), 0, st, a, w, y, g, slab, shift, ep);
-  } else {
+  } else if constexpr (EPI < 2) {
     const dim3 grid = conv_grid((g.M + kBM - 1) / kBM, g.NC / 64, nclasses, k1);
     hipLaunchKernelGGL((conv_tap_k<MODE, 128, 64, 4, 1, 3, EPI, kCT, 32>), grid, dim3(kCT), 0, st, a, w, y, g, slab, shift, ep);
+  } else {
+    std::abort();
   }
 }
 
@@ -1690,6 +1808,29 @@
   else launch_conv_tap<kFwd1>(xp, wp, yp, g, st, stats_slab, stats_shift);
 }
 
+bool conv1x1_recompute_ok(int64_t M, int Cin, int Cout) {
+  return Cin % 64 == 0 && Cin <= 128 && Cout % 128 == 0 && M > 0 && M < ((int64_t)1 << 31) &&
+         !conv1x1_g4w(M, Cin, Cout, 1);
+}
+void conv1x1_stats_only(const void* x, const void* w, int N, int H, int W, int Cin, int Cout,
+                        float* slab, const float* shift, hipStream_t st) {
+  const ConvGeom g{H, W, H, W, 1, H, W, 1, Cin, Cout, N * H * W, Cin};
+  launch_conv_tap<kFwd1, 2>(static_cast<const bf16_t*>(x), static_cast<const bf16_t*>(w), nullptr,
+                            g, st, slab, shift);
+}
+void conv1x1_bn_apply(const void* x, const void* w, void* x3, int N, int H, int W, int Cin,
+                      int Cout, const ConvBnEpi& ep, hipStream_t st) {
+  const ConvGeom g{H, W, H, W, 1, H, W, 1, Cin, Cout, N * H * W, Cin};
+  launch_conv_tap<kFwd1, 3>(static_cast<const bf16_t*>(x), static_cast<const bf16_t*>(w),
+                            static_cast<bf16_t*>(x3), g, st, nullptr, nullptr, ep);
+}
+void conv1x1_bn_bwd(const void* x, const void* w, void* dx, int N, int H, int W, int Cin,
+                    int Cout, const ConvBnEpi& ep, hipStream_t st) {
+  const ConvGeom g{H, W, H, W, 1, H, W, 1, Cin, Cout, N * H * W, Cin};
+  launch_conv_tap<kFwd1, 4>(static_cast<const bf16_t*>(x), static_cast<const bf16_t*>(w),
+                            static_cast<bf16_t*>(dx), g, st, nullptr, nullptr, ep);
+}
+
 int conv_bnbwd_mtiles(int N, int H, int W, int Cout, int ksize, int Cin) {
   const int64_t M = (int64_t)N * H * W;
   if (ksize == 1 && Cout % 128 == 0 && M >= 50176 && Cin < 256) return (int)((M + 63) / 64);
diff --git a/csrc/include/amd_kernels.h b/csrc/include/amd_kernels.h
--- a/csrc/include/amd_kernels.h
+++ b/csrc/include/amd_kernels.h
@@ -258,10 +258,22 @@
   const float* b;
   int relu_mode;
   int add_s2;
+  void* out2;
+  uint8_t* rmask_out;
+  const float* sum_dy;
+  const float* sum_dy_xmu;
+  float inv_n;
 };
 void conv_nhwc_fwd_bnbwd(const void* dy, const void* w, void* g, int N, int H, int W, int Cin,
                          int Cout, int ksize, int stride, const ConvBnEpi& ep, float* slab,
                          hipStream_t st);
+bool conv1x1_recompute_ok(int64_t M, int Cin, int Cout);
+void conv1x1_stats_only(const void* x, const void* w, int N, int H, int W, int Cin, int Cout,
+                        float* slab, const float* shift, hipStream_t st);
+void conv1x1_bn_apply(const void* x, const void* w, void* x3, int N, int H, int W, int Cin,
+                      int Cout, const ConvBnEpi& ep, hipStream_t st);
+void conv1x1_bn_bwd(const void* x, const void* w, void* dx, int N, int H, int W, int Cin,
+                    int Cout, const ConvBnEpi& ep, hipStream_t st);
 void bn_slab_train_stats(const float* slab, int S, int64_t C, int64_t count, const float* shift,
                          float* mean, float* invstd, float* running_mean, float* running_var,
                          long long* nbt, float eps, float momentum, hipStream_t st);
diff --git a/csrc/include/bn_common.h b/csrc/include/bn_common.h
--- a/csrc/include/bn_common.h
+++ b/csrc/include/bn_common.h
@@ -29,6 +29,24 @@
   float is = invstd[c];
   sc = is * w;
   sh = b - mean[c] * sc;
+}
+
+__device__ __forceinline__ float bn_apply_z(float x, float sc, float sh, float z) {
+  float o = fmaf(x, sc, sh);
+  o += z;
+  return o;
+}
+__device__ __forceinline__ float bn_bwd_elem(float dy, float x, float k1, float k2, float k3) {
+  return fmaf(dy, k1, fmaf(x, k2, k3));
+}
+__device__ __forceinline__ void bn_bwd_consts(float is, float wc, float mu, float sum_dy,
+                                              float sum_dy_xmu, float inv_n, float& q1,
+                                              float& q2, float& q3) {
+  const float mdy = sum_dy * inv_n, mdyx = sum_dy_xmu * inv_n;
+  const float a = is * wc, b = -is * is * is * wc * mdyx;
+  q1 = a;
+  q2 = b;
+  q3 = -is * wc * mdy - b * mu;
 }
 
 template <typename TW>
diff --git a/csrc/torch/module.cpp b/csrc/torch/module.cpp
--- a/csrc/torch/module.cpp
+++ b/csrc/torch/module.cpp
@@ -149,6 +149,16 @@
            py::arg("add_stride2") = false);
   conv.def("conv_fwd_stats", &conv_nhwc_fwd_stats_op, py::arg("x"), py::arg("w"),
            py::arg("stride") = 1, py::arg("shift") = py::none());
+  conv.def("recompute_1x1_ok", &conv1x1_recompute_ok_op, py::arg("M"), py::arg("Cin"),
+           py::arg("Cout"));
+  conv.def("conv1x1_stats_only", &conv1x1_stats_only_op, py::arg("x"), py::arg("w"),
+           py::arg("shift") = py::none());
+  conv.def("conv1x1_bn_apply", &conv1x1_bn_apply_op, py::arg("x"), py::arg("w"), py::arg("x3"),
+           py::arg("mean"), py::arg("invstd"), py::arg("bn_weight"), py::arg("bn_bias"),
+           py::arg("z"));
+  conv.def("conv1x1_bn_bwd", &conv1x1_bn_bwd_op, py::arg("x"), py::arg("w"), py::arg("g"),
+           py::arg("mean"), py::arg("invstd"), py::arg("bn_weight"), py::arg("sum_dy"),
+           py::arg("sum_dy_xmu"), py::arg("count"));
   conv.def("conv_dgrad_s2", &conv_nhwc_dgrad_s2_op);
   conv.def("conv_dgrad_s2_bnbwd", &conv_nhwc_dgrad_s2_bnbwd_op, py::arg("dy"), py::arg("wt"),
            py::arg("H"), py::arg("W"), py::arg("x"), py::arg("rmask"), py::arg("mean"),
diff --git a/csrc/torch/pool_ops.cpp b/csrc/torch/pool_ops.cpp
--- a/csrc/torch/pool_ops.cpp
+++ b/csrc/torch/pool_ops.cpp
@@ -163,6 +163,100 @@
   conv_nhwc_fwd(x.data_ptr(), w.data_ptr(), y.data_ptr(), (int)N, (int)H, (int)W, (int)Cin,
                 (int)Cout, (int)k, (int)stride, cur_stream(), slab.data_ptr<float>(), sp);
   return {y, slab};
+}
+
+namespace {
+struct Rec1x1 {
+  int64_t N, Cin, H, W, Cout;
+};
+Rec1x1 rec1x1_check(at::Tensor& x, at::Tensor& w, const char* what) {
+  TORCH_CHECK(x.is_cuda() && x.dim() == 4 && w.dim() == 4 && w.is_cuda(), what,
+              ": 4-D GPU tensors expected");
+  TORCH_CHECK(x.scalar_type() == at::kBFloat16 && w.scalar_type() == at::kBFloat16, what,
+              ": bf16 only");
+  Rec1x1 r{x.size(0), x.size(1), x.size(2), x.size(3), w.size(0)};
+  TORCH_CHECK(w.size(1) == r.Cin && w.size(2) == 1 && w.size(3) == 1, what, ": 1x1 weight");
+  TORCH_CHECK(conv1x1_recompute_ok(r.N * r.H * r.W, (int)r.Cin, (int)r.Cout), what,
+              ": needs Cin 64 | 128, Cout % 128 == 0 and the own-kernel route");
+  x = x.contiguous(at::MemoryFormat::ChannelsLast);
+  w = w.contiguous(at::MemoryFormat::ChannelsLast);
+  return r;
+}
+const float* rec_vec(const at::Tensor& t, int64_t C, const char* what) {
+  TORCH_CHECK(t.is_cuda() && t.scalar_type() == at::kFloat && t.is_contiguous() && t.numel() == C,
+              "conv1x1 recompute: ", what, " must be a contiguous fp32 [C] GPU tensor");
+  return t.data_ptr<float>();
+}
+void rec_like_out(const at::Tensor& t, const Rec1x1& r, const char* what) {
+  TORCH_CHECK(t.is_cuda() && t.dim() == 4 && t.size(0) == r.N && t.size(1) == r.Cout &&
+                  t.size(2) == r.H && t.size(3) == r.W && t.scalar_type() == at::kBFloat16 &&
+                  t.is_contiguous(at::MemoryFormat::ChannelsLast) &&
+                  (uintptr_t)t.data_ptr() % 16 == 0,
+              "conv1x1 recompute: ", what,
+              " must be a channels-last bf16 tensor shaped like the conv output");
+}
+}
+
+bool conv1x1_recompute_ok_op(int64_t M, int64_t Cin, int64_t Cout) {
+  return conv1x1_recompute_ok(M, (int)Cin, (int)Cout);
+}
+
+std::tuple<at::Tensor, at::Tensor> conv1x1_stats_only_op(at::Tensor x, at::Tensor w,
+                                                         c10::optional<at::Tensor> shift) {
+  c10::NoGradGuard no_grad_;
+  const Rec1x1 r = rec1x1_check(x, w, "conv1x1_stats_only");
+  const float* sp = nullptr;
+  if (shift.has_value() && shift->defined()) sp = rec_vec(*shift, r.Cout, "shift");
+  at::Tensor y = at::empty({r.N, r.Cout, r.H, r.W},
+                           x.options().memory_format(at::MemoryFormat::ChannelsLast));
+  const int S = conv_fwd_mtiles((int)r.N, (int)r.H, (int)r.W, (int)r.Cout, 1, 1, (int)r.Cin);
+  at::Tensor slab = at::empty({2, r.Cout, S}, x.options().dtype(at::kFloat));
+  conv1x1_stats_only(x.data_ptr(), w.data_ptr(), (int)r.N, (int)r.H, (int)r.W, (int)r.Cin,
+                     (int)r.Cout, slab.data_ptr<float>(), sp, cur_stream());
+  return {y, slab};
+}
+
+std::tuple<at::Tensor, at::Tensor> conv1x1_bn_apply_op(at::Tensor x, at::Tensor w, at::Tensor x3,
+                                                       at::Tensor mean, at::Tensor invstd,
+                                                       at::Tensor bn_w, at::Tensor bn_b,
+                                                       at::Tensor z) {
+  c10::NoGradGuard no_grad_;
+  const Rec1x1 r = rec1x1_check(x, w, "conv1x1_bn_apply");
+  rec_like_out(x3, r, "x3");
+  rec_like_out(z, r, "z");
+  ConvBnEpi ep{};
+  ep.mean = rec_vec(mean, r.Cout, "mean");
+  ep.invstd = rec_vec(invstd, r.Cout, "invstd");
+  ep.w = rec_vec(bn_w, r.Cout, "weight");
+  ep.b = rec_vec(bn_b, r.Cout, "bias");
+  ep.add = z.data_ptr();
+  at::Tensor y = at::empty_like(x3);
+  at::Tensor mask = at::empty({r.N * r.H * r.W, r.Cout / 8}, x.options().dtype(at::kByte));
+  ep.out2 = y.data_ptr();
+  ep.rmask_out = mask.data_ptr<uint8_t>();
+  conv1x1_bn_apply(x.data_ptr(), w.data_ptr(), x3.data_ptr(), (int)r.N, (int)r.H, (int)r.W,
+                   (int)r.Cin, (int)r.Cout, ep, cur_stream());
+  return {y, mask};
+}
+
+at::Tensor conv1x1_bn_bwd_op(at::Tensor x, at::Tensor w, at::Tensor g, at::Tensor mean,
+                             at::Tensor invstd, at::Tensor bn_w, at::Tensor sum_dy,
+                             at::Tensor sum_dy_xmu, double count) {
+  c10::NoGradGuard no_grad_;
+  const Rec1x1 r = rec1x1_check(x, w, "conv1x1_bn_bwd");
+  rec_like_out(g, r, "g");
+  ConvBnEpi ep{};
+  ep.mean = rec_vec(mean, r.Cout, "mean");
+  ep.invstd = rec_vec(invstd, r.Cout, "invstd");
+  ep.w = rec_vec(bn_w, r.Cout, "weight");
+  ep.sum_dy = rec_vec(sum_dy, r.Cout, "sum_dy");
+  ep.sum_dy_xmu = rec_vec(sum_dy_xmu, r.Cout, "sum_dy_xmu");
+  ep.inv_n = (float)(1.0 / count);
+  ep.add = g.data_ptr();
+  at::Tensor dx = at::empty_like(g);
+  conv1x1_bn_bwd(x.data_ptr(), w.data_ptr(), dx.data_ptr(), (int)r.N, (int)r.H, (int)r.W,
+                 (int)r.Cin, (int)r.Cout, ep, cur_stream());
+  return dx;
 }
 
 std::tuple<at::Tensor, at::Tensor> conv_nhwc_fwd_bnbwd_op(
diff --git a/csrc/torch/pool_ops.h b/csrc/torch/pool_ops.h
--- a/csrc/torch/pool_ops.h
+++ b/csrc/torch/pool_ops.h
@@ -24,6 +24,16 @@
     c10::optional<at::Tensor> rmask, at::Tensor mean, at::Tensor invstd,
     c10::optional<at::Tensor> bn_w, c10::optional<at::Tensor> bn_b, int64_t relu_mode,
     bool add_stride2 = false);
+bool conv1x1_recompute_ok_op(int64_t M, int64_t Cin, int64_t Cout);
+std::tuple<at::Tensor, at::Tensor> conv1x1_stats_only_op(at::Tensor x, at::Tensor w,
+                                                         c10::optional<at::Tensor> shift);
+std::tuple<at::Tensor, at::Tensor> conv1x1_bn_apply_op(at::Tensor x, at::Tensor w, at::Tensor x3,
+                                                       at::Tensor mean, at::Tensor invstd,
+                                                       at::Tensor bn_w, at::Tensor bn_b,
+                                                       at::Tensor z);
+at::Tensor conv1x1_bn_bwd_op(at::Tensor x, at::Tensor w, at::Tensor g, at::Tensor mean,
+                             at::Tensor invstd, at::Tensor bn_w, at::Tensor sum_dy,
+                             at::Tensor sum_dy_xmu, double count);
 at::Tensor conv_nhwc_dgrad_s2_op(at::Tensor dy, at::Tensor wt, int64_t H, int64_t W);
 at::Tensor conv_nhwc_wgrad_op(at::Tensor dy, at::Tensor x, at::ScalarType out_dtype, int64_t algo,
                               int64_t stride, int64_t ksize, c10::optional<at::Tensor> out, bool accumulate = true);
```

New measurement: 12880 images/s (median of 6 runs). 1.1% higher.
